# peaceminusones/Group-GAN-GCN-GAT

Measured on AMD Instinct MI355X. Metric: scenes/sec (obs8/pred12, 20 peds) at 1/2/4/8 GPUs; ADE/FDE vs ref, higher is better.
Workload: dtype fp32; 1 GPU; train iteration = D-step + G-step (best_k=20, Adam), GAT generator; BASELINE configs[1] shape (batch 64); scenes_per_gpu=64, global_batch=64, obs_len=8, pred_len=12, generator=gat, hip_graph=True, parallelism=dp1

## Files before the change

### group-gan-gcn-gat_amd/csrc/adam.hip

```cpp
#include "sgg_common.h"

namespace sgg {

constexpr int kAdamMaxTensors = 48;
constexpr int kAdamThreads = 256;
constexpr int kAdamChunk = 1024;

struct AdamList {
  float* p[kAdamMaxTensors];
  float* g[kAdamMaxTensors];
  float* m[kAdamMaxTensors];
  float* v[kAdamMaxTensors];
  float* step[kAdamMaxTensors];
  long long off[kAdamMaxTensors + 1];
  int n;
};

__device__ __forceinline__ float block_sum(float x, float* red) {
  for (int o = 32; o > 0; o >>= 1) x += __shfl_xor(x, o);
  const int lane = threadIdx.x & 63, wave = threadIdx.x >> 6;
  if (lane == 0) red[wave] = x;
  __syncthreads();
  float s = 0.f;
#pragma unroll
  for (int w = 0; w < kAdamThreads / 64; ++w) s += red[w];
  __syncthreads();
  return s;
}

constexpr int kAdamPer = kAdamChunk / kAdamThreads;

struct Tab {
  long long lo, hi;
  unsigned long long p, g, m, v;
};

__device__ __forceinline__ Tab lane_tab(const AdamList& L) {
  const int t = threadIdx.x & 63;
  Tab r = {0, 0, 0, 0, 0, 0};
  if (t < L.n) {
    r.lo = L.off[t];
    r.hi = L.off[t + 1];
    r.p = reinterpret_cast<unsigned long long>(L.p[t]);
    r.g = reinterpret_cast<unsigned long long>(L.g[t]);
    r.m = reinterpret_cast<unsigned long long>(L.m[t]);
    r.v = reinterpret_cast<unsigned long long>(L.v[t]);
  }
  return r;
}

__device__ __forceinline__ long long rl64(long long x, int k) {
  const int lo = __builtin_amdgcn_readlane((int)(unsigned)(unsigned long long)x, k);
  const int hi = __builtin_amdgcn_readlane((int)(unsigned)((unsigned long long)x >> 32), k);
  return (long long)(((unsigned long long)(unsigned)hi << 32) | (unsigned)lo);
}
__device__ __forceinline__ unsigned long long shfl64(unsigned long long x, int k) {
  const unsigned lo = (unsigned)__shfl((int)(unsigned)x, k), hi = (unsigned)__shfl((int)(unsigned)(x >> 32), k);
  return ((unsigned long long)hi << 32) | lo;
}

__device__ __forceinline__ void chunk_elems(const AdamList& L, const Tab& T, long long e0, int (&ek)[kAdamPer],
                                            long long (&ei)[kAdamPer]) {
  const long long total = L.off[L.n];
  const long long e1 = (e0 + kAdamChunk < total ? e0 + kAdamChunk : total) - 1;
  const int t = threadIdx.x & 63;
  const unsigned long long b0 = __ballot(t < L.n && T.lo <= e0 && e0 < T.hi);
  const unsigned long long b1 = __ballot(t < L.n && T.lo <= e1 && e1 < T.hi);
  const int k0 = b0 ? __ffsll((long long)b0) - 1 : 0, k1 = b1 ? __ffsll((long long)b1) - 1 : k0;
#pragma unroll
  for (int u = 0; u < kAdamPer; ++u) {
    ek[u] = -1;
    ei[u] = 0;
  }
  for (int k = k0; k <= k1; ++k) {
    const long long lo = rl64(T.lo, k), hi = rl64(T.hi, k);
#pragma unroll
    for (int u = 0; u < kAdamPer; ++u) {
      const long long e = e0 + threadIdx.x + (long long)u * kAdamThreads;
      if (e >= lo && e < hi) {
        ek[u] = k;
        ei[u] = e - lo;
      }
    }
  }
}

__global__ void __launch_bounds__(kAdamThreads) adam_prep_kernel(AdamList L, int clip, float* __restrict__ partial,
                                                                 float* __restrict__ scal, double lr, double beta1,
                                                                 double beta2) {
  __shared__ float red[kAdamThreads / 64];
  if (blockIdx.x == 0 && (int)threadIdx.x < L.n) {
    const float t = L.step[threadIdx.x][0] + 1.f;
    L.step[threadIdx.x][0] = t;
    scal[2 * threadIdx.x] = (float)(lr / (1.0 - pow(beta1, (double)t)));
    scal[2 * threadIdx.x + 1] = (float)sqrt(1.0 - pow(beta2, (double)t));
  }
  if (!clip) return;
  const long long e0 = (long long)blockIdx.x * kAdamChunk;
  const Tab T = lane_tab(L);
  int ek[kAdamPer];
  long long ei[kAdamPer];
  chunk_elems(L, T, e0, ek, ei);
  float x[kAdamPer];
#pragma unroll
  for (int u = 0; u < kAdamPer; ++u) {
    const float* g = reinterpret_cast<const float*>(shfl64(T.g, ek[u] < 0 ? 0 : ek[u]));
    x[u] = ek[u] >= 0 ? g[ei[u]] : 0.f;
  }
  float acc = 0.f;
#pragma unroll
  for (int u = 0; u < kAdamPer; ++u) acc = fmaf(x[u], x[u], acc);
  const float s = block_sum(acc, red);
  if (threadIdx.x == 0) partial[blockIdx.x] = s;
}

__global__ void __launch_bounds__(kAdamThreads) adam_update_kernel(AdamList L, int nparts, float max_norm,
                                                                   const float* __restrict__ partial,
                                                                   const float* __restrict__ scal, float beta2,
                                                                   float w1, float w2, float eps,
                                                                   unsigned* __restrict__ ticket, double lr,
                                                                   double beta1d, double beta2d) {
  __shared__ float red[kAdamThreads / 64];
  __shared__ int last;
  const long long e0 = (long long)blockIdx.x * kAdamChunk;
  const Tab T = lane_tab(L);
  float tstep = 0.f, lss = 0.f, lbc = 1.f;
  if (ticket && (int)(threadIdx.x & 63) < L.n) {
    tstep = L.step[threadIdx.x & 63][0] + 1.f;
    lss = (float)(lr / (1.0 - pow(beta1d, (double)tstep)));
    lbc = (float)sqrt(1.0 - pow(beta2d, (double)tstep));
  }
  int ek[kAdamPer];
  long long ei[kAdamPer];
  chunk_elems(L, T, e0, ek, ei);
  float coef = 1.f;
  if (max_norm > 0.f) {
    float acc = 0.f;
    for (int q = threadIdx.x; q < nparts; q += kAdamThreads) acc += partial[q];
    const float norm = sqrtf(block_sum(acc, red));
    coef = fminf(max_norm / (norm + 1e-6f), 1.f);
  }
  float* pp[kAdamPer];
  float* gp[kAdamPer];
  float* mp[kAdamPer];
  float* vp[kAdamPer];
  float gr[kAdamPer], m0[kAdamPer], v0[kAdamPer], p0[kAdamPer], ss[kAdamPer], bc[kAdamPer];
#pragma unroll
  for (int u = 0; u < kAdamPer; ++u) {
    const int k = ek[u] >= 0 ? ek[u] : 0;
    const long long i = ek[u] >= 0 ? ei[u] : 0;
    pp[u] = reinterpret_cast<float*>(shfl64(T.p, k)) + i;
    gp[u] = reinterpret_cast<float*>(shfl64(T.g, k)) + i;
    mp[u] = reinterpret_cast<float*>(shfl64(T.m, k)) + i;
    vp[u] = reinterpret_cast<float*>(shfl64(T.v, k)) + i;
    if (ticket) {
      ss[u] = __shfl(lss, k);
      bc[u] = __shfl(lbc, k);
    } else {
      ss[u] = scal[2 * k];
      bc[u] = scal[2 * k + 1];
    }
  }
#pragma unroll
  for (int u = 0; u < kAdamPer; ++u) {
    gr[u] = *gp[u];
    m0[u] = *mp[u];
    v0[u] = *vp[u];
    p0[u] = *pp[u];
  }
#pragma unroll
  for (int u = 0; u < kAdamPer; ++u) {
    if (ek[u] < 0) continue;
    float g = gr[u];
    if (max_norm > 0.f) {
      g *= coef;
      *gp[u] = g;
    }
    const float mi = m0[u] + w1 * (g - m0[u]);
    const float vi = v0[u] * beta2 + w2 * g * g;
    *mp[u] = mi;
    *vp[u] = vi;
    *pp[u] = p0[u] + -ss[u] * (mi / (sqrtf(vi) / bc[u] + eps));
  }
  if (ticket) {
    __syncthreads();
    if (threadIdx.x == 0) last = atomicAdd(ticket, 1u) == gridDim.x - 1;
    __syncthreads();
    if (last) {
      if ((int)threadIdx.x < L.n) L.step[threadIdx.x][0] = tstep;
      if (threadIdx.x == 0) *ticket = 0u;
    }
  }
}

}

using namespace sgg;

extern "C" int sgg_adam_parts(long long total) {
  return (int)((total + kAdamChunk - 1) / kAdamChunk) + 2 * kAdamMaxTensors + 1;
}

extern "C" int sgg_adam_step(float* const* params, float* const* grads, float* const* exp_avg,
                             float* const* exp_avg_sq, const long long* numel, int n, double lr, double beta1,
                             double beta2, float eps, float max_norm, float* const* step, float* ws,
                             size_t ws_bytes, void* stream) {
  SGG_CHECK_ARG(params && grads && exp_avg && exp_avg_sq && numel && step, "sgg_adam_step: null pointer");
  SGG_CHECK_ARG(n >= 1 && n <= kAdamMaxTensors, "sgg_adam_step: %d tensors (1..%d)", n, kAdamMaxTensors);
  AdamList L;
  L.n = n;
  L.off[0] = 0;
  for (int i = 0; i < n; ++i) {
    SGG_CHECK_ARG(params[i] && grads[i] && exp_avg[i] && exp_avg_sq[i] && step[i] && numel[i] >= 0,
                  "sgg_adam_step: tensor %d", i);
    L.p[i] = params[i];
    L.g[i] = grads[i];
    L.m[i] = exp_avg[i];
    L.v[i] = exp_avg_sq[i];
    L.step[i] = step[i];
    L.off[i + 1] = L.off[i] + numel[i];
  }
  const int parts = sgg_adam_parts(L.off[n]) - 2 * kAdamMaxTensors - 1;
  if (parts == 0) return 0;
  const int clip = max_norm > 0.f;
  SGG_CHECK_ARG(ws && ws_bytes >= sizeof(float) * ((size_t)parts + 2 * kAdamMaxTensors + 1),
                "sgg_adam_step: workspace");
  hipStream_t st = (hipStream_t)stream;
  unsigned* ticket = reinterpret_cast<unsigned*>(ws);
  float* partial = ws + 1;
  float* scal = partial + parts;
  if (clip)
    hipLaunchKernelGGL(adam_prep_kernel, dim3(parts), dim3(kAdamThreads), 0, st, L, clip, partial, scal, lr, beta1,
                       beta2);
  hipLaunchKernelGGL(adam_update_kernel, dim3(parts), dim3(kAdamThreads), 0, st, L, parts, clip ? max_norm : 0.f,
                     partial, scal, (float)beta2, (float)(1.0 - beta1), (float)(1.0 - beta2), eps, clip ? nullptr : ticket,
                     lr, beta1, beta2);
  SGG_RETURN_LAUNCH("sgg_adam_step");
}
```

### group-gan-gcn-gat_amd/csrc/fold.hip

```cpp
#include "sgg_common.h"

namespace sgg {

__global__ void __launch_bounds__(512) fold_fwd_kernel(const float* __restrict__ W, int ldw, int R, int E,
                                                       const float* __restrict__ We, const float* __restrict__ be,
                                                       const float* __restrict__ b1, const float* __restrict__ b2,
                                                       float* __restrict__ A, float* __restrict__ bias) {
  for (int r = threadIdx.x; r < R; r += blockDim.x) {
    float a0 = 0.f, a1 = 0.f, bb = 0.f;
    const float* w = W + (size_t)r * ldw;
#pragma unroll 8
    for (int e = 0; e < E; ++e) {
      const float we = w[e];
      a0 = fmaf(we, We[2 * e], a0);
      a1 = fmaf(we, We[2 * e + 1], a1);
      bb = fmaf(we, be[e], bb);
    }
    A[2 * r] = a0;
    A[2 * r + 1] = a1;
    bias[r] = bb + b1[r] + (b2 ? b2[r] : 0.f);
  }
}

struct FoldList {
  SggFold f[SGG_FOLD_MAX];
};

__global__ void __launch_bounds__(512) fold_fwd_multi_kernel(FoldList L) {
  const SggFold& d = L.f[blockIdx.x];
  for (int r = threadIdx.x; r < d.R; r += blockDim.x) {
    float a0 = 0.f, a1 = 0.f, bb = 0.f;
    const float* w = d.W + (size_t)r * d.ldw;
#pragma unroll 8
    for (int e = 0; e < d.E; ++e) {
      const float we = w[e];
      a0 = fmaf(we, d.We[2 * e], a0);
      a1 = fmaf(we, d.We[2 * e + 1], a1);
      bb = fmaf(we, d.be[e], bb);
    }
    d.A[2 * r] = a0;
    d.A[2 * r + 1] = a1;
    d.bias[r] = bb + d.b1[r] + (d.b2 ? d.b2[r] : 0.f);
  }
}

__device__ __forceinline__ void fold_bwd_body(const float* __restrict__ W, int ldw, int R, int E,
                                              const float* __restrict__ We, const float* __restrict__ be,
                                              const float* __restrict__ dA, const float* __restrict__ dbias,
                                              float* __restrict__ dW, int lddw, float* __restrict__ dWe,
                                              float* __restrict__ dbe, float* __restrict__ dbias_copy) {
  __shared__ float g3[3 * 512];
  __shared__ float part[3 * 512];
  for (int r = threadIdx.x; r < R; r += blockDim.x) {
    const float2 a = reinterpret_cast<const float2*>(dA)[r];
    const float b = dbias[r];
    g3[3 * r] = a.x;
    g3[3 * r + 1] = a.y;
    g3[3 * r + 2] = b;
    if (dbias_copy) dbias_copy[r] = b;
  }
  __syncthreads();
  const int ng = blockDim.x / E;
  const int t = threadIdx.x;
  if (t < ng * E) {
    const int e = t % E, g = t / E;
    const float we0 = We[2 * e], we1 = We[2 * e + 1], bee = be[e];
    float s0 = 0.f, s1 = 0.f, s2 = 0.f;
#pragma unroll 8
    for (int r = g; r < R; r += ng) {
      const float a0 = g3[3 * r], a1 = g3[3 * r + 1], b = g3[3 * r + 2];
      dW[(size_t)r * lddw + e] = fmaf(a0, we0, fmaf(a1, we1, b * bee));
      const float w = W[(size_t)r * ldw + e];
      s0 = fmaf(w, a0, s0);
      s1 = fmaf(w, a1, s1);
      s2 = fmaf(w, b, s2);
    }
    part[3 * t] = s0;
    part[3 * t + 1] = s1;
    part[3 * t + 2] = s2;
  }
  __syncthreads();
  if (t < 3 * E) {
    const int e = t / 3, j = t - 3 * e;
    float s = 0.f;
    for (int g = 0; g < ng; ++g) s += part[3 * (g * E + e) + j];
    if (j < 2) dWe[2 * e + j] = s;
    else dbe[e] = s;
  }
}

__global__ void __launch_bounds__(512) fold_bwd_kernel(const float* __restrict__ W, int ldw, int R, int E,
                                                       const float* __restrict__ We, const float* __restrict__ be,
                                                       const float* __restrict__ dA, const float* __restrict__ dbias,
                                                       float* __restrict__ dW, int lddw, float* __restrict__ dWe,
                                                       float* __restrict__ dbe, float* __restrict__ dbias_copy) {
  fold_bwd_body(W, ldw, R, E, We, be, dA, dbias, dW, lddw, dWe, dbe, dbias_copy);
}

struct FoldBwdList {
  SggFoldBwd f[SGG_FOLDB_MAX];
};

__global__ void __launch_bounds__(512) fold_bwd_multi_kernel(FoldBwdList L) {
  const SggFoldBwd& d = L.f[blockIdx.x];
  fold_bwd_body(d.W, d.ldw, d.R, d.E, d.We, d.be, d.dA_src, d.db_src, d.dW, d.lddw, d.dWe, d.dbe, d.dbias_copy);
}

void fold_bwd_multi(const SggFoldBwd* folds, int n, hipStream_t st) {
  FoldBwdList L;
  for (int k = 0; k < n; ++k) L.f[k] = folds[k];
  hipLaunchKernelGGL(fold_bwd_multi_kernel, dim3(n), dim3(512), 0, st, L);
}

}

using namespace sgg;

extern "C" int sgg_fold_fwd(const float* W, int ldw, int R, int E, const float* We, const float* be, const float* b1,
                            const float* b2, float* A, float* bias, void* stream) {
  SGG_CHECK_ARG(W && We && be && b1 && A && bias, "sgg_fold_fwd: null pointer");
  SGG_CHECK_ARG(R >= 1 && E >= 1 && ldw >= E, "sgg_fold_fwd: bad sizes R=%d E=%d ldw=%d", R, E, ldw);
  hipLaunchKernelGGL(fold_fwd_kernel, dim3(1), dim3(512), 0, (hipStream_t)stream, W, ldw, R, E, We, be, b1, b2, A,
                     bias);
  SGG_RETURN_LAUNCH("sgg_fold_fwd");
}

extern "C" int sgg_fold_fwd_multi(const SggFold* folds, int n, void* stream) {
  SGG_CHECK_ARG(folds && n >= 1 && n <= SGG_FOLD_MAX, "sgg_fold_fwd_multi: 1 <= n <= %d folds (got %d)", SGG_FOLD_MAX, n);
  FoldList L;
  for (int k = 0; k < n; ++k) {
    const SggFold& d = folds[k];
    SGG_CHECK_ARG(d.W && d.We && d.be && d.b1 && d.A && d.bias, "sgg_fold_fwd_multi: null pointer in fold %d", k);
    SGG_CHECK_ARG(d.R >= 1 && d.E >= 1 && d.ldw >= d.E, "sgg_fold_fwd_multi: bad sizes in fold %d", k);
    L.f[k] = d;
  }
  hipLaunchKernelGGL(fold_fwd_multi_kernel, dim3(n), dim3(512), 0, (hipStream_t)stream, L);
  SGG_RETURN_LAUNCH("sgg_fold_fwd_multi");
}

extern "C" int sgg_fold_bwd(const float* W, int ldw, int R, int E, const float* We, const float* be, const float* dA,
                            const float* dbias, float* dW, int lddw, float* dWe, float* dbe, float* dbias_copy,
                            void* stream) {
  SGG_CHECK_ARG(W && We && be && dA && dbias && dW && dWe && dbe, "sgg_fold_bwd: null pointer");
  SGG_CHECK_ARG(R >= 1 && R <= 512 && E >= 1 && E <= 128 && ldw >= E && lddw >= E, "sgg_fold_bwd: bad sizes");
  hipLaunchKernelGGL(fold_bwd_kernel, dim3(1), dim3(512), 0, (hipStream_t)stream, W, ldw, R, E, We, be, dA, dbias,
                     dW, lddw, dWe, dbe, dbias_copy);
  SGG_RETURN_LAUNCH("sgg_fold_bwd");
}
```

### group-gan-gcn-gat_amd/csrc/grad.hip

```cpp
#include <string.h>

#include "bce_body.h"
#include "sgg_common.h"

namespace sgg {

namespace {

constexpr int kRedJobs = SGG_RED_MAX + 2 * SGG_FOLDB_MAX;

struct FinishArgs {
  SggRed red[kRedJobs];
  unsigned char vec[kRedJobs];
  int nred;
  int blk0[kRedJobs + 1];
  SggL2Job l2[SGG_LOSSJOB_MAX];
  SggBceJob bce[SGG_LOSSJOB_MAX];
  int nl2, nbce;
};

__device__ __forceinline__ float phase_sum(const float* __restrict__ src, int rows, int ld, int col, int ph) {
  float s = 0.f;
  int r = ph;
  for (; r + 48 < rows; r += 64) {
    const float v0 = src[(size_t)r * ld + col], v1 = src[(size_t)(r + 16) * ld + col];
    const float v2 = src[(size_t)(r + 32) * ld + col], v3 = src[(size_t)(r + 48) * ld + col];
    s += v0;
    s += v1;
    s += v2;
    s += v3;
  }
  for (; r < rows; r += 16) s += src[(size_t)r * ld + col];
  return s;
}

__device__ __forceinline__ floatx4 phase_sum4(const float* __restrict__ src, int rows, int ld, int col, int ph) {
  floatx4 s = {0.f, 0.f, 0.f, 0.f};
  int r = ph;
  for (; r + 48 < rows; r += 64) {
    const floatx4 v0 = *reinterpret_cast<const floatx4*>(src + (size_t)r * ld + col);
    const floatx4 v1 = *reinterpret_cast<const floatx4*>(src + (size_t)(r + 16) * ld + col);
    const floatx4 v2 = *reinterpret_cast<const floatx4*>(src + (size_t)(r + 32) * ld + col);
    const floatx4 v3 = *reinterpret_cast<const floatx4*>(src + (size_t)(r + 48) * ld + col);
    s += v0;
    s += v1;
    s += v2;
    s += v3;
  }
  for (; r < rows; r += 16) s += *reinterpret_cast<const floatx4*>(src + (size_t)r * ld + col);
  return s;
}

__device__ __forceinline__ void red_store(const SggRed& d, int c, float v) {
  if (d.map == 0) {
    d.out[c] = v;
  } else {
    const int m = c / d.N, n = c - m * d.N;
    d.out[d.trans ? (size_t)n * d.ldo + m : (size_t)m * d.ldo + n] = v;
  }
}

__device__ void red_job(const SggRed& d, bool vec, int blk, float (*rpart)[256]) {
  const int el = threadIdx.x & 63, ph = threadIdx.x >> 6;
  if (vec) {
    const int c = blk * 256 + 4 * el;
    const floatx4 s = c < d.cols ? phase_sum4(d.src + d.col0, d.rows, d.ld, c, ph) : floatx4{0.f, 0.f, 0.f, 0.f};
    *reinterpret_cast<floatx4*>(&rpart[ph][4 * el]) = s;
    __syncthreads();
    if (ph == 0 && c < d.cols) {
      floatx4 v = {0.f, 0.f, 0.f, 0.f};
#pragma unroll
      for (int p = 0; p < 16; ++p) v += *reinterpret_cast<const floatx4*>(&rpart[p][4 * el]);
#pragma unroll
      for (int i = 0; i < 4; ++i)
        if (c + i < d.cols) red_store(d, c + i, v[i]);
    }
    return;
  }
  const int c = blk * 64 + el;
  const float s = c < d.cols ? phase_sum(d.src + d.col0, d.rows, d.ld, c, ph) : 0.f;
  rpart[ph][el] = s;
  __syncthreads();
  if (ph == 0 && c < d.cols) {
    float v = 0.f;
#pragma unroll
    for (int p = 0; p < 16; ++p) v += rpart[p][el];
    red_store(d, c, v);
  }
}

constexpr int kLossThreads = 1024;

__device__ void l2_value(const SggL2Job& d, float* lv) {
  if (threadIdx.x < 64) {
    float a = 0.f;
    for (int s = threadIdx.x; s < d.S; s += 64) a += d.term[s];
    a = wave_sum(a);
    if (threadIdx.x == 0) {
      *d.loss = a;
      *lv = a;
    }
  }
  __syncthreads();
}

static_assert(kLossThreads == kBceThreads, "the loss workgroup runs bce_value with its own thread count");

__device__ void loss_workgroup(const FinishArgs& a, float (*rpart)[256]) {
  __shared__ float lv[SGG_LOSSJOB_MAX];
  BceIn in[SGG_LOSSJOB_MAX];
#pragma unroll
  for (int j = 0; j < SGG_LOSSJOB_MAX; ++j)
    if (j < a.nbce) bce_load(a.bce[j], in[j]);
  float ad[SGG_LOSSJOB_MAX];
#pragma unroll
  for (int j = 0; j < SGG_LOSSJOB_MAX; ++j) {
    ad[j] = 0.f;
    if (j < a.nbce && a.bce[j].total) {
      bool fromL2 = false;
      for (int k = 0; k < a.nl2; ++k) fromL2 |= a.bce[j].addend == a.l2[k].loss;
      if (!fromL2) ad[j] = *a.bce[j].addend;
    }
  }
  for (int k = 0; k < a.nl2; ++k) l2_value(a.l2[k], lv + k);
#pragma unroll
  for (int j = 0; j < SGG_LOSSJOB_MAX; ++j)
    if (j < a.nbce) {
      float addend = ad[j];
      for (int k = 0; k < a.nl2; ++k)
        if (a.bce[j].total && a.bce[j].addend == a.l2[k].loss) addend = lv[k];
      bce_value(a.bce[j], in[j], addend, reinterpret_cast<float(*)[kLossThreads / 64]>(&rpart[0][0]));
    }
}

__global__ void __launch_bounds__(1024) grad_finish_kernel(FinishArgs a) {
  __shared__ __attribute__((aligned(16))) float rpart[16][256];
  const int lw = a.nl2 + a.nbce > 0;
  const int b = (int)blockIdx.x - lw;
  if (b < 0) {
    loss_workgroup(a, rpart);
    return;
  }
  int j = 0;
  while (j + 1 < a.nred && b >= a.blk0[j + 1]) ++j;
  red_job(a.red[j], a.vec[j] != 0, b - a.blk0[j], rpart);
}

}

}

using namespace sgg;

extern "C" int sgg_grad_finish(const SggRed* reds, int nred, const SggFoldBwd* folds, int nfold, float* scratch,
                               size_t scratch_bytes, void* stream) {
  return sgg_grad_finish_losses(reds, nred, folds, nfold, scratch, scratch_bytes, nullptr, 0, nullptr, 0, stream);
}

extern "C" int sgg_grad_finish_losses(const SggRed* reds, int nred, const SggFoldBwd* folds, int nfold,
                                      float* scratch, size_t scratch_bytes, const SggL2Job* l2, int nl2,
                                      const SggBceJob* bce, int nbce, void* stream) {
  SGG_CHECK_ARG(nl2 >= 0 && nl2 <= SGG_LOSSJOB_MAX && nbce >= 0 && nbce <= SGG_LOSSJOB_MAX &&
                    (nl2 == 0 || l2) && (nbce == 0 || bce),
                "sgg_grad_finish_losses: 0 <= nl2, nbce <= %d (got %d, %d)", SGG_LOSSJOB_MAX, nl2, nbce);
  for (int j = 0; j < nl2; ++j) {
    const SggL2Job& d = l2[j];
    SGG_CHECK_ARG(d.loss && (d.S == 0 || d.term) && d.S >= 0, "sgg_grad_finish_losses: bad L2 job %d", j);
  }
  for (int j = 0; j < nbce; ++j) {
    const SggBceJob& d = bce[j];
    SGG_CHECK_ARG(d.ya && d.yb && d.loss && (d.n == 0 || d.x) && (!d.total || d.addend),
                  "sgg_grad_finish_losses: null pointer in BCE job %d", j);
    SGG_CHECK_ARG(d.n >= 0 && d.split >= 0 && d.split <= d.n, "sgg_grad_finish_losses: BCE job %d: bad sizes", j);
  }
  SGG_CHECK_ARG(nred >= 0 && nred <= SGG_RED_MAX && nfold >= 0 && nfold <= SGG_FOLDB_MAX,
                "sgg_grad_finish: 0 <= nred <= %d, 0 <= nfold <= %d (got %d, %d)", SGG_RED_MAX, SGG_FOLDB_MAX, nred,
                nfold);
  SGG_CHECK_ARG((nred == 0 || reds) && (nfold == 0 || (folds && scratch)), "sgg_grad_finish: null job list or scratch");
  FinishArgs a;
  memset(&a, 0, sizeof(a));
  int nj = 0;
  auto add_red = [&](const SggRed& d) {
    a.red[nj] = d;
    ++nj;
  };
  for (int j = 0; j < nred; ++j) {
    const SggRed& d = reds[j];
    SGG_CHECK_ARG(d.src && d.out && d.rows >= 0 && d.cols >= 1 && d.col0 >= 0 && d.ld >= d.col0 + d.cols,
                  "sgg_grad_finish: bad reduction job %d (rows %d ld %d col0 %d cols %d)", j, d.rows, d.ld, d.col0,
                  d.cols);
    SGG_CHECK_ARG(d.map == 0 || (d.map == 1 && d.N >= 1 && d.cols % d.N == 0 &&
                                 d.ldo >= (d.trans ? d.cols / d.N : d.N)),
                  "sgg_grad_finish: bad output map of reduction job %d", j);
    add_red(d);
  }
  size_t need = 0;
  for (int k = 0; k < nfold; ++k) need += sizeof(float) * 3 * (size_t)folds[k].R;
  SGG_CHECK_ARG(scratch_bytes >= need, "sgg_grad_finish: scratch %zu < %zu bytes", scratch_bytes, need);
  float* g = scratch;
  for (int k = 0; k < nfold; ++k) {
    const SggFoldBwd& d = folds[k];
    SGG_CHECK_ARG(d.W && d.We && d.be && d.dA_src && d.db_src && d.dW && d.dWe && d.dbe,
                  "sgg_grad_finish: null pointer in fold job %d", k);
    SGG_CHECK_ARG(d.R >= 1 && d.R <= 512 && d.E >= 1 && d.E <= 128 && d.ldw >= d.E && d.lddw >= d.E,
                  "sgg_grad_finish: bad fold sizes in job %d (R %d E %d)", k, d.R, d.E);
    SGG_CHECK_ARG(d.dA_rows >= 0 && d.db_rows >= 0 && d.dA_col0 >= 0 && d.db_col0 >= 0 &&
                      d.dA_ld >= d.dA_col0 + 2 * d.R && d.db_ld >= d.db_col0 + d.R,
                  "sgg_grad_finish: bad (dA, dbias) sources in fold job %d", k);
    add_red(SggRed{d.dA_src, d.dA_rows, d.dA_ld, d.dA_col0, 2 * d.R, g, 0, 0, 0, 0});
    add_red(SggRed{d.db_src, d.db_rows, d.db_ld, d.db_col0, d.R, g + 2 * d.R, 0, 0, 0, 0});
    g += 3 * (size_t)d.R;
  }
  a.nred = nj;
  int blk = 0;
  for (int j = 0; j < nj; ++j) {
    const SggRed& d = a.red[j];
    a.vec[j] = d.ld % 4 == 0 && d.col0 % 4 == 0 && (reinterpret_cast<uintptr_t>(d.src) & 15) == 0;
    a.blk0[j] = blk;
    blk += a.vec[j] ? (d.cols + 255) / 256 : (d.cols + 63) / 64;
  }
  a.blk0[nj] = blk;
  for (int j = 0; j < nl2; ++j) a.l2[j] = l2[j];
  for (int j = 0; j < nbce; ++j) a.bce[j] = bce[j];
  a.nl2 = nl2;
  a.nbce = nbce;
  if (nl2 + nbce > 0) ++blk;
  hipStream_t st = (hipStream_t)stream;
  if (blk > 0) hipLaunchKernelGGL(grad_finish_kernel, dim3(blk), dim3(1024), 0, st, a);
  if (nfold > 0) {
    SggFoldBwd f[SGG_FOLDB_MAX];
    g = scratch;
    for (int k = 0; k < nfold; ++k) {
      f[k] = folds[k];
      f[k].dA_src = g;
      f[k].db_src = g + 2 * folds[k].R;
      g += 3 * (size_t)folds[k].R;
    }
    fold_bwd_multi(f, nfold, st);
  }
  SGG_RETURN_LAUNCH("sgg_grad_finish");
}
```

### group-gan-gcn-gat_amd/sgan/_native.py

```python
import ctypes
import os

import torch

from ._srchash import source_hash

_LIB_EXPLICIT = bool(os.environ.get("SGG_LIB"))
_LIB_PATH = os.environ.get("SGG_LIB") or os.path.join(os.path.dirname(os.path.abspath(__file__)), "_lib", "libsgg.so")

_i = ctypes.c_int
_f = ctypes.c_float
_p = ctypes.c_void_p
_sz = ctypes.c_size_t
_u = ctypes.c_uint
_u64 = ctypes.c_ulonglong

MAX_HEADS = 4


class GatEncWeights(ctypes.Structure):
    _fields_ = [("Wi", _p * MAX_HEADS), ("ai", _p * MAX_HEADS), ("Wio", _p), ("aio", _p),
                ("Wg", _p * MAX_HEADS), ("ag", _p * MAX_HEADS), ("Wgo", _p), ("ago", _p), ("Woe", _p), ("boe", _p)]


class GatEncArgs(ctypes.Structure):
    _fields_ = [("X", _p), ("ldx", _i), ("labels", _p), ("scene_off", _p), ("S", _i), ("np", _i), ("nh", _i),
                ("alpha", _f), ("w", GatEncWeights), ("y", _p), ("ldy", _i), ("dy", _p), ("lddy", _i), ("dX", _p),
                ("lddx", _i), ("slab", _p), ("saved", _p), ("X2", _p), ("ldx2", _i), ("kx1", _i),
                ("dX2", _p), ("lddx2", _i), ("dy_copies", _i), ("dy_cstride", _i)]


_pargs = ctypes.POINTER(GatEncArgs)


class GcnModArgs(ctypes.Structure):
    _fields_ = [("X", _p), ("ldx", _i), ("X2", _p), ("ldx2", _i), ("kx1", _i), ("labels", _p), ("scene_off", _p),
                ("S", _i), ("np", _i), ("fin", _i), ("fe", _i), ("bf16", _i), ("W0i", _p), ("W1i", _p), ("W0g", _p),
                ("W1g", _p), ("Woe", _p), ("boe", _p), ("y", _p), ("ldy", _i), ("dy", _p), ("lddy", _i),
                ("dy_copies", _i), ("dy_cstride", _i), ("dX", _p), ("lddx", _i), ("dX2", _p), ("lddx2", _i),
                ("slab", _p)]


_gargs = ctypes.POINTER(GcnModArgs)


class LstmSeg(ctypes.Structure):
    _fields_ = [("rel", _p), ("A", _p), ("Whh", _p), ("bias", _p), ("h0", _p), ("c0", _p), ("T", _i), ("B", _i),
                ("Bl", _i), ("t0", _i), ("Tl", _i), ("Bsrc", _i), ("h_all", _p), ("c_all", _p), ("act_all", _p),
                ("Wu", _p), ("ldwu", _i), ("cu", _p), ("NU", _i), ("U", _p)]


_sargs = ctypes.POINTER(LstmSeg)


class PoolDh(ctypes.Structure):
    _fields_ = [("dU", _p), ("ldu", _i), ("W1h", _p), ("ldw", _i), ("base", _p), ("NU", _i), ("h", _p), ("ldh", _i),
                ("ws", _p), ("ws_bytes", _sz), ("splits", _i)]


GLUE_NONE, GLUE_SELECT, GLUE_L2BWD = 0, 1, 2


class GlueSeg(ctypes.Structure):
    _fields_ = [("kind", _i), ("pred", _p), ("ldp", _i), ("gt", _p), ("mask", _p), ("ldm", _i), ("scene_off", _p),
                ("S", _i), ("T", _i), ("B", _i), ("k", _i), ("best", _p), ("w", _f), ("gout", _p), ("dpred", _p),
                ("ldd", _i), ("term", _p)]

FOLD_MAX = 8


class Fold(ctypes.Structure):
    _fields_ = [("W", _p), ("ldw", _i), ("R", _i), ("E", _i), ("We", _p), ("be", _p), ("b1", _p), ("b2", _p),
                ("A", _p), ("bias", _p)]

RED_MAX = 24
FOLDB_MAX = 6


class Red(ctypes.Structure):
    _fields_ = [("src", _p), ("rows", _i), ("ld", _i), ("col0", _i), ("cols", _i), ("out", _p), ("map", _i),
                ("N", _i), ("ldo", _i), ("trans", _i)]


class FoldBwd(ctypes.Structure):
    _fields_ = [("W", _p), ("ldw", _i), ("R", _i), ("E", _i), ("We", _p), ("be", _p),
                ("dA_src", _p), ("dA_rows", _i), ("dA_ld", _i), ("dA_col0", _i),
                ("db_src", _p), ("db_rows", _i), ("db_ld", _i), ("db_col0", _i),
                ("dW", _p), ("lddw", _i), ("dWe", _p), ("dbe", _p), ("dbias_copy", _p)]


class DecInit(ctypes.Structure):
    _fields_ = [("ctx", _p), ("ldc", _i), ("Dc", _i), ("z", _p), ("nz", _i), ("best", _p), ("first_k", _i),
                ("ped_scene", _p), ("S", _i), ("Bper", _i), ("last_rel", _p)]


LOSSJOB_MAX = 2


class TrajOut(ctypes.Structure):
    _fields_ = [("out", _p), ("NB", _i), ("T0", _i), ("col0", _i), ("ncol", _i), ("head", _p), ("ldh", _i),
                ("b", _p), ("ldb", _i), ("pos0", _p), ("start", _p)]


class PoolBatch(ctypes.Structure):
    _fields_ = [("U", _p), ("pos", _p), ("scene_off", _p), ("chunks", _p), ("nchunks", _i), ("max_rows", _i),
                ("gpw", _i), ("B", _i), ("max_n", _i), ("out", _p), ("argmax", _p), ("nchunks_dev", _p)]


class GatLayerSet(ctypes.Structure):
    _fields_ = [("x1", _p), ("ld1", _i), ("K1", _i), ("x2", _p), ("ld2", _i), ("K2", _i), ("seg_off", _p),
                ("nseg", _i), ("n", _i), ("max_seg", _i), ("xn", _p), ("rstd", _p), ("wh", _p), ("hp", _p), ("y", _p),
                ("ldy", _i)]


class L2Job(ctypes.Structure):
    _fields_ = [("term", _p), ("S", _i), ("loss", _p)]


class BceJob(ctypes.Structure):
    _fields_ = [("x", _p), ("n", _i), ("split", _i), ("ya", _p), ("yb", _p), ("w", _f), ("loss", _p),
                ("addend", _p), ("total", _p), ("nvalid", _p)]


class DecStep(ctypes.Structure):
    _fields_ = ([(n, _i) for n in ("B", "H", "bn", "mlp_dim", "NU", "mlp", "cell", "ldwu")]
                + [(n, _p) for n in ("h_prev", "pool_prev", "c_prev", "r_in", "pos_prev",
                                     "W1m", "b1m", "W2m", "b2m", "A", "Whh", "bias", "Wp", "bp", "Wu", "cu",
                                     "h", "c", "rel", "pos", "U", "act", "h_mix", "z1")])


class DecStepBwd(ctypes.Structure):
    _fields_ = ([(n, _i) for n in ("B", "H", "bn", "mlp_dim", "mlp", "cell")]
                + [(n, _p) for n in ("dh", "dc", "drel", "dpos", "act", "c", "c_prev", "h_mix", "z1",
                                     "W1m", "W2m", "A", "Whh", "Wp",
                                     "dh_prev", "dpool_prev", "dc_prev", "dr_in", "dpos_prev",
                                     "dG", "dz2", "dz1", "drel_tot")])


SIGNATURES = {
    "sgg_version": (_i, []),
    "sgg_last_error": (ctypes.c_char_p, []),
    "sgg_source_hash": (ctypes.c_char_p, []),
    "sgg_xw": (_i, [_p, _i, _p, _i, _p, _i, _i, _p, _p, _i, _i, _i, _i, _i, _p]),
    "sgg_xw_bf16": (_i, [_p, _i, _p, _i, _p, _i, _i, _p, _p, _i, _i, _i, _i, _i, _p]),
    "sgg_pool_plan": (_i, [_p, _i, _i, _i, _i, _p, _i, _p, _p]),
    "sgg_pool_fwd": (_i, [_p, _p, _p, _p, _p, _p, _p, _i, _i, _i, _i, _i, _i, _p, _p, _p, _p]),
    "sgg_pool_plan_bf16": (_i, [_p, _i, _i, _i, _p, _i, _p, _p]),
    "sgg_pool_fwd_bf16": (_i, [_p, _p, _p, _p, _p, _p, _p, _i, _i, _i, _i, _i, _i, _p, _p, _p, _p]),
    "sgg_pool_fwd2": (_i, [ctypes.POINTER(PoolBatch), ctypes.POINTER(PoolBatch), _p, _p, _p, _i, _i, _p]),
    "sgg_pool_bwd_grid": (_i, [_i]),
    "sgg_pool_dh_dw": (_i, [_p, _i, _p, _i, _p, _i, _i, _p, _i, _i, _i, _p, _sz, _p]),
    "sgg_pool_bwd": (_i, [_p, _p, _p, _p, _p, _p, _p, _p, _i, _i, _i, _i, _p, _p, _p]),
    "sgg_pool_plan_wide": (_i, [_p, _i, _i, _i, _p, _i, _p, _p]),
    "sgg_pool_fwd_wide": (_i, [_p, _p, _p, _p, _p, _p, _p, _i, _i, _i, _i, _i, _i, _p, _p, _p]),
    "sgg_pool_bwd_wide_grid": (_i, [_i, _i]),
    "sgg_pool_bwd_wide": (_i, [_p, _p, _p, _p, _p, _p, _p, _p, _i, _i, _i, _i, _p, _p, _p]),
    "sgg_pool_plan_bn": (_i, [_p, _i, _i, _i, _p, _i, _p, _p]),
    "sgg_pool_fwd_bn": (_i, [_p, _p, _p, _p, _p, _p, _p, _i, _i, _i, _i, _i, _i, _p, _p, _p]),
    "sgg_pool_bwd_bn_grid": (_i, [_i, _i, _i]),
    "sgg_pool_bwd_bn_ws_floats": (ctypes.c_longlong, [_i, _i, _i, _i]),
    "sgg_pool_bwd_bn": (_i, [_p, _p, _p, _p, _p, _p, _p, _p, _i, _i, _i, _i, _p, _p, _sz, _p]),
    "sgg_gat_fwd": (_i, [_p, _i, _p, _p, _p, _p, _i, _i, _i, _f, _i, _i, _i, _p, _p, _i, _p]),
    "sgg_gat_bwd": (_i, [_p, _i, _p, _p, _p, _i, _i, _i, _f, _i, _i, _i, _p, _p, _p, _i, _p, _p, _p, _p]),
    "sgg_gat_fwd_ex": (_i, [_p, _i, _p, _p, _p, _p, _p, _i, _i, _i, _f, _i, _i, _i, _p, _p, _i, _p]),
    "sgg_gat_bwd_ex": (_i, [_p, _i, _p, _p, _p, _p, _i, _i, _i, _f, _i, _i, _i, _p, _p, _p, _i, _p, _p, _p, _p, _p,
                            _p]),
    "sgg_gat_bwd_ex_work_bytes": (_sz, [_i, _i, _i]),
    "sgg_gat_wide_work_floats": (_sz, [_i, _i, _i, _i, _i]),
    "sgg_gat_fwd_wide": (_i, [_p, _i, _p, _p, _i, _p, _p, _p, _i, _i, _i, _f, _i, _i, _i, _p, _p, _i, _p, _p]),
    "sgg_gat_bwd_wide": (_i, [_p, _i, _p, _p, _i, _p, _p, _i, _i, _i, _f, _i, _i, _i, _p, _p, _p, _i, _p, _p, _p, _p,
                              _p, _p, _p, _p]),
    "sgg_gat_fwd_drop": (_i, [_p, _i, _p, _p, _i, _p, _p, _p, _i, _i, _i, _f, _i, _i, _i, _p, _p, _i,
                              _f, _u64, _u, _u, _u, _p, _p]),
    "sgg_gat_bwd_drop": (_i, [_p, _i, _p, _p, _i, _p, _p, _i, _i, _i, _f, _i, _i, _i, _p, _p, _p, _i, _p, _p, _p, _p,
                              _p, _p, _p, _f, _u64, _u, _u, _u, _p, _p]),
    "sgg_dropout": (_i, [_p, _i, _i, _i, _f, _u64, _u, _u, _p, _p, _i, _p]),
    "sgg_gat_layer_lds_bytes": (_sz, [_i, _i, _i]),
    "sgg_gat_layer_fwd": (_i, [_p, _i, _i, _p, _i, _i, _p, _p, _p, _p, _p, _i, _i, _i, _i, _f, _f, _i, _i, _i, _p, _p,
                               _p, _p, _p, _i, _p]),
    "sgg_gat_layer_fwd2": (_i, [ctypes.POINTER(GatLayerSet), ctypes.POINTER(GatLayerSet), _p, _p, _p, _p, _i, _i, _f,
                                _f, _i, _i, _p]),
    "sgg_seg_norm_fwd": (_i, [_p, _i, _i, _p, _i, _f, _p, _i, _p, _p]),
    "sgg_seg_norm_bwd": (_i, [_p, _i, _p, _i, _i, _p, _i, _p, _p, _i, _p]),
    "sgg_group_index_ws": (_sz, [_i, _i]),
    "sgg_group_index": (_i, [_p, _p, _i, _i, _i, _p, _p, _p, _p, _p, _p, _p]),
    "sgg_seg_reduce": (_i, [_p, _i, _i, _p, _p, _p, _p, _p, _i, _i, _p, _i, _p]),
    "sgg_seg_gather": (_i, [_p, _i, _i, _p, _p, _p, _i, _p, _i, _p]),
    "sgg_xtw_splits": (_i, [_i, _i, _i]),
    "sgg_lstm_bwd_split": (_i, [_p, _p, _p, _p, _p, _p, _p, _p, _p, _p, _i, _i, _i, _i, _p, _p, _p, _p, _p]),
    "sgg_lstm_bwd_tail": (_i, [_p, _p, _p, _p, _p, _p, _p, _i, _i, _i, _i, _p, _p]),
    "sgg_lstm_fwd_seg": (_i, [_sargs, _i, _p]),
    "sgg_lstm_fwd_seg_glue": (_i, [_sargs, _i, ctypes.POINTER(GlueSeg), _p]),
    "sgg_lstm_fwd_seg2": (_i, [_sargs, _i, _sargs, _i, _p]),
    "sgg_lstm_fwd_seg3": (_i, [_sargs, _i, _sargs, _i, _sargs, _i, _p]),
    "sgg_lstm_bwd_shared": (_i, [_p, _p, _p, _p, _p, _p, _p, _i, _i, _i, _i, _i, _p, _p, _p]),
    "sgg_lstm_bwd_pooldh_ok": (_i, [_i]),
    "sgg_lstm_bwd_pooldh_pays": (_i, [_i, _i]),
    "sgg_lstm_bwd_pooldh_rides": (_i, [_i, _i, _i]),
    "sgg_lstm_bwd_pooldh": (_i, [_p, _p, _p, _p, _p, _p, ctypes.POINTER(PoolDh), _i, _i, _i, _i, _i, _i, _p, _p, _p,
                                 _p]),
    "sgg_lstm_u_ok": (_i, [_i, _i, _i, _i, _i, _i]),
    "sgg_lstm_fwd_u": (_i, [_p, _p, _p, _p, _p, _p, _i, _i, _i, _p, _p, _p, _p, _i, _p, _i, _p, _p]),
    "sgg_head_ok": (_i, [_i, _i]),
    "sgg_head_slab_cols": (_i, [_i, _i]),
    "sgg_head_fwd": (_i, [_p, _i, _i, _i, _i, _p, _p, _p, _p, _i, _p, _p, _p]),
    "sgg_head_bwd": (_i, [_p, _i, _i, _i, _i, _p, _p, _p, _p, _p, _i, _p, _i, _p, _p, _p, _p, _i, _f, _p, _p]),
    "sgg_head_fwdbwd": (_i, [_p, _i, _i, _i, _i, _p, _p, _p, _p, _i, _p, _p, _i, _p, _p, _p, _p, _i, _f, _p, _p]),
    "sgg_xtw_partial": (_i, [_p, _i, _p, _i, _p, _i, _i, _i, _i, _i, _p, _sz, _p]),
    "sgg_grad_finish": (_i, [ctypes.POINTER(Red), _i, ctypes.POINTER(FoldBwd), _i, _p, _sz, _p]),
    "sgg_lstm_fwd_dec": (_i, [ctypes.POINTER(DecInit), _p, _p, _p, _p, _p, _i, _i, _i, _p, _p, _p, _p, _p,
                              ctypes.POINTER(TrajOut), _p]),
    "sgg_lstm_fwd_dec2": (_i, [ctypes.POINTER(DecInit), ctypes.POINTER(DecInit), _p, _p, _p, _p, _p, _i, _i, _i, _i,
                               _p, _p, ctypes.POINTER(TrajOut), _p]),
    "sgg_lstm_fwd_dec_seg": (_i, [ctypes.POINTER(DecInit), _p, _p, _p, _p, _p, _i, _i, _i, _p, _p, _p, _p, _p,
                                  ctypes.POINTER(TrajOut), _sargs, _i, _p]),
    "sgg_grad_finish_losses": (_i, [ctypes.POINTER(Red), _i, ctypes.POINTER(FoldBwd), _i, _p, _sz,
                                    ctypes.POINTER(L2Job), _i, ctypes.POINTER(BceJob), _i, _p]),
    "sgg_adam_parts": (_i, [ctypes.c_longlong]),
    "sgg_adam_step": (_i, [_p, _p, _p, _p, _p, _i, ctypes.c_double, ctypes.c_double, ctypes.c_double, _f, _f, _p, _p,
                          _sz, _p]),
    "sgg_xtw": (_i, [_p, _i, _p, _i, _p, _i, _i, _i, _i, _p, _i, _i, _p, _p, _sz, _p]),
    "sgg_fold_fwd": (_i, [_p, _i, _i, _i, _p, _p, _p, _p, _p, _p, _p]),
    "sgg_fold_fwd_multi": (_i, [ctypes.POINTER(Fold), _i, _p]),
    "sgg_fold_bwd": (_i, [_p, _i, _i, _i, _p, _p, _p, _p, _p, _i, _p, _p, _p, _p]),
    "sgg_lstm_fwd": (_i, [_p, _p, _p, _p, _p, _p, _p, _p, _i, _i, _i, _i, _p, _p, _p, _p, _p]),
    "sgg_lstm_state_floats": (ctypes.c_longlong, [_i, _i, _i, _i]),
    "sgg_lstm_dg_floats": (ctypes.c_longlong, [_i, _i, _i]),
    "sgg_lstm_wpart_rows": (_i, [_i, _i]),
    "sgg_lstm_kernel_name": (ctypes.c_char_p, [_i, _i, _i, _i, _i]),
    "sgg_lstm_bwd": (_i, [_p, _p, _p, _p, _p, _p, _p, _p, _p, _p, _i, _i, _i, _i, _p, _p, _p, _p, _p, _p]),
    "sgg_bce_fwd": (_i, [_p, _i, _i, _p, _p, _f, _p, _p, _p, _p, _p]),
    "sgg_bce_bwd": (_i, [_p, _i, _i, _p, _p, _f, _p, _p, _p, _p]),
    "sgg_gatenc_param_size": (_i, [_i]),
    "sgg_gatenc_lds_bytes": (ctypes.c_longlong, [_i, _i, _i]),
    "sgg_gatenc_saved_floats": (ctypes.c_longlong, [_i, _i, _i]),
    "sgg_gatenc_fwd": (_i, [_pargs, _p]),
    "sgg_gatenc_fwd2": (_i, [_pargs, _pargs, _p]),
    "sgg_gatenc_bwd": (_i, [_pargs, _p]),
    "sgg_gcnmod_param_size": (_i, [_i, _i]),
    "sgg_gcnmod_slab_rows": (_i, [_i]),
    "sgg_gcnmod_lds_bytes": (ctypes.c_longlong, [_i, _i, _i, _i]),
    "sgg_gcnmod_fwd": (_i, [_gargs, _p]),
    "sgg_gcnmod_fwd2": (_i, [_gargs, _gargs, _p]),
    "sgg_gcnmod_bwd": (_i, [_gargs, _p]),
    "sgg_slab_reduce": (_i, [_p, _i, _i, _p, _p]),
    "sgg_gather_batch_floats": (ctypes.c_longlong, [_i, _i, _i]),
    "sgg_gather_batch": (_i, [_p, _i, _p, _i, _i, _i, _p, _p]),
    "sgg_traj_cat": (_i, [_p, _i, _i, _p, _i, _p, _i, _i, _i, _p, _p, _p, _p]),
    "sgg_decoder_init": (_i, [_p, _i, _i, _p, _i, _p, _i, _i, _p, _i, _i, _p, _p, _p, _p]),
    "sgg_l2_select": (_i, [_p, _p, _p, _i, _p, _i, _i, _i, _i, _p, _p]),
    "sgg_l2_loss_fwd": (_i, [_p, _i, _p, _p, _i, _p, _i, _i, _i, _f, _p, _p, _p, _p]),
    "sgg_l2_loss_bwd": (_i, [_p, _i, _p, _p, _i, _p, _p, _i, _i, _f, _p, _p, _i, _p]),
    "sgg_l2_loss_bwd_scenes": (_i, [_p, _i, _p, _p, _i, _p, _i, _i, _i, _f, _p, _p, _i, _p, _p]),
    "sgg_val_metrics_work_floats": (_sz, [_i]),
    "sgg_val_metrics": (_i, [_p, _p, _p, _p, _p, _i, _p, _p, _f, _i, _i, _p, _p, _p]),
    "sgg_dec_step_ok": (_i, [_i, _i, _i, _i]),
    "sgg_dec_step_saved_floats": (ctypes.c_longlong, [_i, _i, _i]),
    "sgg_dec_step_fwd": (_i, [ctypes.POINTER(DecStep), _p]),
    "sgg_dec_step_bwd": (_i, [ctypes.POINTER(DecStepBwd), _p]),
    "sgg_pool_dpos": (_i, [_p, _p, _p, _p, _p, _p, _p, _p, _i, _i, _i, _p, _p]),
    "sgg_pool_fwd_bn_drop": (_i, [_p, _p, _p, _p, _p, _p, _p, _i, _i, _i, _i, _i, _i, _p, _p, _f, _u64, _u, _p, _p]),
    "sgg_pool_bwd_bn_drop": (_i, [_p, _p, _p, _p, _p, _p, _p, _p, _i, _i, _i, _i, _p, _p, _sz, _f, _u64, _u, _p, _p]),
    "sgg_pool_dpos_drop": (_i, [_p, _p, _p, _p, _p, _p, _p, _p, _i, _i, _i, _p, _f, _u64, _u, _p, _p]),
    "sgg_pool_norm_fwd": (_i, [_p] * 10 + [_i] * 5 + [_f, _f] + [_p] * 9),
    "sgg_pool_norm_running": (_i, [_p, _p, _p, _i, _i, _f, _p, _p, _p]),
    "sgg_pool_norm_bwd_rows": (_i, [_i]),
    "sgg_pool_norm_bwd_ws_floats": (ctypes.c_longlong, [_i, _i, _i]),
    "sgg_pool_norm_bwd_slab_offset": (ctypes.c_longlong, [_i, _i]),
    "sgg_pool_norm_bwd": (_i, [_p] * 18 + [_i] * 5 + [_f, _f, _i, _p, _p, _p, _sz, _p]),
}

VAL_SLOTS = 11

_lib = None


class NativeError(RuntimeError):
    pass


def lib_path():
    return _LIB_PATH


def built_hash():
    return load(require_gpu=False).sgg_source_hash().decode()


def load(require_gpu=True):
    global _lib
    if _lib is None:
        if not os.path.exists(_LIB_PATH):
            raise NativeError("libsgg.so not built at %s -- run group-gan-gcn-gat_amd/build_native.py "
                              "(or __graft_entry__.build())" % _LIB_PATH)
        lib = ctypes.CDLL(_LIB_PATH)
        for name, (res, args) in SIGNATURES.items():
            fn = getattr(lib, name)
            fn.restype = res
            fn.argtypes = args
        if not _LIB_EXPLICIT:
            built, tree = lib.sgg_source_hash().decode(), source_hash()
            if built != tree:
                raise NativeError("%s was built from other sources (hash %s) than this tree's csrc/ + "
                                  "include/sgg.h (%s) -- rebuild with group-gan-gcn-gat_amd/build_native.py"
                                  % (_LIB_PATH, built[:16], tree[:16]))
        _lib = lib
    if require_gpu and not torch.cuda.is_available():
        raise NativeError("sgan: no HIP device visible; the MI355X kernels have no CPU fallback")
    return _lib


def check(rc, name):
    if rc != 0:
        msg = _lib.sgg_last_error().decode(errors="replace")
        raise NativeError("%s failed (rc=%d): %s" % (name, rc, msg))


def stream_ptr():
    return ctypes.c_void_p(torch.cuda.current_stream().cuda_stream)


def ptr(t):
    if t is None:
        return None
    return ctypes.c_void_p(t.data_ptr())
```

### group-gan-gcn-gat_amd/sgan/kernels.py

```python
import collections
import contextlib
import ctypes
import functools
import os
import weakref

import torch

from . import _native as N

GATENC_FUSED = os.environ.get("SGG_GATENC_FUSED", "1") != "0"
GATENC_SAVE = os.environ.get("SGG_GATENC_SAVE", "1") != "0"
DUAL_POOL_BWD = os.environ.get("SGG_DUAL_POOL_BWD", "1") != "0"
POOL_DH_IN_LSTM = os.environ.get("SGG_POOL_DH_IN_LSTM", "1") != "0"


DEBUG = os.environ.get("SGG_DEBUG", "0") == "1"


def _lib():
    return N.load()


def _req(t, name, dtype=torch.float32):
# ... 46 lines not shown
    import ctypes
    dev = torch.cuda.current_device() if device is None else torch.device(device).index
    if dev is None:
        dev = torch.cuda.current_device()
    key = (tag, dev)
    st = _private.get(key)
    if st is None:
        if _hiprt is None:
            lib = ctypes.CDLL(os.path.join(os.path.dirname(torch.__file__), "lib", "libamdhip64.so"))
            lib.hipStreamCreateWithFlags.argtypes = [ctypes.POINTER(ctypes.c_void_p), ctypes.c_uint]
            lib.hipStreamCreateWithFlags.restype = ctypes.c_int
            _hiprt = lib
        h = ctypes.c_void_p()
        with torch.cuda.device(dev):
            rc = _hiprt.hipStreamCreateWithFlags(ctypes.byref(h), 1)
        if rc != 0 or not h.value:
            raise N.NativeError("hipStreamCreateWithFlags failed (%d)" % rc)
        st = _private[key] = torch.cuda.ExternalStream(h.value, device=torch.device("cuda", dev))
    return st


def xw_raw(x, w, bias=None, trans_w=False, act=0, out=None, mask=None, prec=None):
    x = _rows(x, "x")
    if mask is not None:
        mask = _rows(mask, "mask")
        assert mask.shape == x.shape
    w = _rows(w, "w")
    M, K = x.shape
    Nn = w.shape[0] if trans_w else w.shape[1]
    assert (w.shape[1] if trans_w else w.shape[0]) == K, (x.shape, w.shape, trans_w)
    if bias is not None:
        bias = _req(bias, "bias").contiguous()
        assert bias.numel() == Nn
    y = out if out is not None else torch.empty(M, Nn, device=x.device, dtype=torch.float32)

    bf16 = (prec or _PRECISION) == "bf16"
    fn = _lib().sgg_xw_bf16 if bf16 else _lib().sgg_xw

    def launch():
        N.check(fn(N.ptr(x), x.stride(0), N.ptr(mask), mask.stride(0) if mask is not None else 0,
                   N.ptr(w), w.stride(0), int(bool(trans_w)), N.ptr(bias), N.ptr(y), y.stride(0), M, K, Nn,
                   int(act), N.stream_ptr()), "sgg_xw")
    launch()
    if timer.active and M > 0:
        tw = "true" if trans_w else "false"
        name = ("sgg::xw_bf16_kernel<%s>" % tw if bf16 else
                "sgg::xw_splitk_kernel<%s>" % tw if K >= 256 else
                "sgg::xw_kernel<true, true>" if trans_w and K <= 256 else
                "sgg::xw_kernel<%s, false>" % tw)
        timer.add(name, (M, K, Nn, mask is not None), 2.0 * M * K * Nn,
                  4.0 * (M * K * (2 if mask is not None else 1) + K * Nn + M * Nn), launch)
    return y


def xtw(X, Y, colsum=False, trans_c=False, out=None, mask=None):
    lib = _lib()
    X = _rows(X, "X")
    Y = _rows(Y, "Y")
    if mask is not None:
        mask = _rows(mask, "mask")
        assert mask.shape == Y.shape
    R, M = X.shape
    Nn = Y.shape[1]
    assert Y.shape[0] == R
    shape = (Nn, M) if trans_c else (M, Nn)
    if out is None:
        C = torch.empty(shape, device=X.device, dtype=torch.float32)
    else:
        assert tuple(out.shape) == shape and out.stride(1) == 1, (out.shape, shape)
        C = out
    if R == 0:
        C.zero_()
        return (C, torch.zeros(Nn, device=X.device)) if colsum else C
    splits = lib.sgg_xtw_splits(R, M, Nn)
    ws = torch.empty(splits * (M * Nn + Nn), device=X.device, dtype=torch.float32)
    cs = torch.empty(Nn, device=X.device, dtype=torch.float32) if colsum else None
    def launch():
        N.check(lib.sgg_xtw(N.ptr(X), X.stride(0), N.ptr(Y), Y.stride(0), N.ptr(mask),
                            mask.stride(0) if mask is not None else 0, R, M, Nn, N.ptr(C), C.stride(0), int(trans_c),
                            N.ptr(cs), N.ptr(ws), ws.numel() * 4, N.stream_ptr()), "sgg_xtw")
    launch()
    if timer.active:
        timer.add("sgg::xtw_partial_kernel+xtw_reduce_kernel", (R, M, Nn, mask is not None), 2.0 * R * M * Nn,
                  4.0 * (R * M + R * Nn * (2 if mask is not None else 1) + M * Nn) + 8.0 * ws.numel(), launch)
    return (C, cs) if colsum else C


def fold_fwd(W, We, be, b1, b2=None):
    key, ver = _fold_key(W, We, be, b1, b2)
    ent = _FOLD_CACHE.get(key)
    if _fold_hit(ent, ver, (W, We, be, b1, b2)):
        return ent[1], ent[2]
    prefold([(W, We, be, b1, b2)])
    ent = _FOLD_CACHE[key]
    return ent[1], ent[2]


_EPOCH = {}
_FOLD_CACHE = {}


def _fold_key(W, We, be, b1, b2):
    ts = (W, We, be, b1, b2)
    key = tuple((t.data_ptr(), tuple(t.shape), t.stride(0)) if t is not None else None for t in ts)
    ver = tuple((t._version, _EPOCH.get(t.data_ptr(), 0)) if t is not None else None for t in ts)
    return key, ver


def _owner(t):
    return t._base if t._base is not None else t


def _fold_hit(ent, ver, ts):
    return (ent is not None and ent[0] == ver
            and all((r is None) if t is None else (r is not None and r() is _owner(t)) for r, t in zip(ent[4], ts)))


def _fold_purge():
    dead = [k for k, e in _FOLD_CACHE.items() if any(r is not None and r() is None for r in e[4])]
    for k in dead:
        del _FOLD_CACHE[k]


def clear_fold_cache():
    _FOLD_CACHE.clear()


def prefold(specs):
    todo = []
    for W, We, be, b1, b2 in specs:
        key, ver = _fold_key(W, We, be, b1, b2)
        if not _fold_hit(_FOLD_CACHE.get(key), ver, (W, We, be, b1, b2)):
            todo.append((key, ver, (W, We, be, b1, b2)))
    if not todo:
        return
    _fold_purge()
    arr = (N.Fold * len(todo))()
    outs = []
    for k, (key, ver, (W, We, be, b1, b2)) in enumerate(todo):
        W = _rows(W, "W")
        R, E = W.shape
        A = torch.empty(R, 2, device=W.device, dtype=torch.float32)
        bias = torch.empty(R, device=W.device, dtype=torch.float32)
        parts = (W, We.contiguous(), be.contiguous(), b1.contiguous(), b2.contiguous() if b2 is not None else None)
        arr[k] = N.Fold(N.ptr(parts[0]), W.stride(0), R, E, N.ptr(parts[1]), N.ptr(parts[2]), N.ptr(parts[3]),
                        N.ptr(parts[4]), N.ptr(A), N.ptr(bias))
        outs.append((key, ver, A, bias, parts))
    for i in range(0, len(todo), N.FOLD_MAX):
        chunk = (N.Fold * min(N.FOLD_MAX, len(todo) - i))(*arr[i:i + N.FOLD_MAX])
        N.check(_lib().sgg_fold_fwd_multi(chunk, len(chunk), N.stream_ptr()), "sgg_fold_fwd_multi")
    for (key, ver, A, bias, parts), (_, _, ts) in zip(outs, todo):
        refs = tuple(weakref.ref(_owner(t)) if t is not None else None for t in ts)
        copies = tuple(p for p, t in zip(parts, ts) if p is not None and p.data_ptr() != t.data_ptr())
        _FOLD_CACHE[key] = (ver, A, bias, copies, refs)


def lstm_fold_spec(lstm, emb):
    return (lstm.weight_ih_l0, emb.weight, emb.bias, lstm.bias_ih_l0, lstm.bias_hh_l0)


def pool_fold_spec(pool):
    l1, E = pool_linears(pool)[0], pool.embedding_dim
    return (l1.weight[:, :E], pool.spatial_embedding.weight, pool.spatial_embedding.bias, l1.bias, None)


def fold_bwd(W, We, be, dA, dbias, dW=None, dbias_copy=None):
    W = _rows(W, "W")
    R, E = W.shape
    dW = dW if dW is not None else torch.empty(R, E, device=W.device, dtype=torch.float32)
    dWe = torch.empty(E, 2, device=W.device, dtype=torch.float32)
    dbe = torch.empty(E, device=W.device, dtype=torch.float32)
    N.check(_lib().sgg_fold_bwd(N.ptr(W), W.stride(0), R, E, N.ptr(We.contiguous()), N.ptr(be.contiguous()),
                                N.ptr(dA.contiguous()), N.ptr(dbias.contiguous()), N.ptr(dW), dW.stride(0), N.ptr(dWe),
                                N.ptr(dbe), N.ptr(dbias_copy), N.stream_ptr()), "sgg_fold_bwd")
    return dW, dWe, dbe


def xtw_partial(X, Y, colsum=False):
    lib = _lib()
    X = _rows(X, "X")
    Y = _rows(Y, "Y")
    R, M = X.shape
    Nn = Y.shape[1]
    assert Y.shape[0] == R and R > 0
    splits = lib.sgg_xtw_splits(R, M, Nn)
    ws = torch.empty(splits * (M * Nn + (Nn if colsum else 0)), device=X.device, dtype=torch.float32)

    def launch():
        N.check(lib.sgg_xtw_partial(N.ptr(X), X.stride(0), N.ptr(Y), Y.stride(0), None, 0, R, M, Nn, int(colsum),
                                    N.ptr(ws), ws.numel() * 4, N.stream_ptr()), "sgg_xtw_partial")
    launch()
    if timer.active:
        mt = 4 if M >= 64 else (M + 15) // 16
        timer.add("sgg::xtw_partial_kernel<%d>" % mt, (R, M, Nn), 2.0 * R * M * Nn,
                  4.0 * (R * M + R * Nn) + 4.0 * ws.numel(), launch)
    return ws, splits


class GradFinish:

    def __init__(self):
        self.reds, self.folds, self.keep = [], [], []

    def _hold(self, *ts):
        self.keep += [t.untyped_storage() for t in ts if t is not None]

    def rowsum(self, src, rows, ld, col0, cols, out):
        assert out.is_contiguous() and out.numel() == cols
        self.reds.append(N.Red(N.ptr(src), rows, ld, col0, cols, N.ptr(out), 0, 0, 0, 0))
        self._hold(src, out)

    def xtw_sums(self, ws, splits, M, Nn, C, trans_c=False, colsum=None):
        assert C.stride(1) == 1 and tuple(C.shape) == ((Nn, M) if trans_c else (M, Nn))
        self.reds.append(N.Red(N.ptr(ws), splits, M * Nn, 0, M * Nn, N.ptr(C), 1, Nn, C.stride(0), int(trans_c)))
        self._hold(ws, C)
        if colsum is not None:
            self.rowsum(ws[splits * M * Nn:], splits, Nn, 0, Nn, colsum)

    def fold(self, W, We, be, dA_src, dA_rows, dA_ld, dA_col0, db_src, db_rows, db_ld, db_col0, dW=None,
             dbias_copy=None):
        W = _rows(W, "W")
        R, E = W.shape
        dW = dW if dW is not None else torch.empty(R, E, device=W.device, dtype=torch.float32)
        dWe = torch.empty(E, 2, device=W.device, dtype=torch.float32)
        dbe = torch.empty(E, device=W.device, dtype=torch.float32)
        We, be = We.contiguous(), be.contiguous()
        self.folds.append(N.FoldBwd(N.ptr(W), W.stride(0), R, E, N.ptr(We), N.ptr(be),
                                    N.ptr(dA_src), dA_rows, dA_ld, dA_col0, N.ptr(db_src), db_rows, db_ld, db_col0,
                                    N.ptr(dW), dW.stride(0), N.ptr(dWe), N.ptr(dbe), N.ptr(dbias_copy)))
        self._hold(W, We, be, dA_src, db_src, dW, dWe, dbe, dbias_copy)
        return dW, dWe, dbe

    def run(self):
        if not self.reds and not self.folds:
            return
        if _DEFER[0] > 0:
            _PENDING.append(self)
            return
        _finish_launch(self.reds, self.folds, self.keep)


_DEFER = [0]
_PENDING = []
_LOSS = {"l2": [], "bce": [], "keep": [], "out": set()}


DEFER_LOSSES = os.environ.get("SGG_DEFER_LOSSES", "1") != "0"


def _loss_deferrable(kind):
    return DEFER_LOSSES and _DEFER[0] > 0 and not _NO_DEFER[0] and len(_LOSS[kind]) < N.LOSSJOB_MAX


@contextlib.contextmanager
def eager_losses():
    prev = _NO_DEFER[0]
    _NO_DEFER[0] = True
    try:
        yield
    finally:
        _NO_DEFER[0] = prev


_NO_DEFER = [False]


def _queue_loss(kind, job, keep, outs):
    _LOSS[kind].append(job)
    _LOSS["keep"] += [t.untyped_storage() for t in keep if t is not None]
    _LOSS["out"].update(t.data_ptr() for t in outs)


def _loss_pending(t):
    return t is not None and t.data_ptr() in _LOSS["out"]


def _take_losses():
    glue_flush()
    l2, bce, keep = _LOSS["l2"], _LOSS["bce"], _LOSS["keep"]
    _LOSS.update(l2=[], bce=[], keep=[], out=set())
    return l2, bce, keep


def flush_losses():
    l2, bce, keep = _take_losses()
    if l2 or bce:
        _finish_launch([], [], keep, l2, bce)


@contextlib.contextmanager
def defer_grad_finish():
    if os.environ.get("SGG_CHECK_DEFER") == "1":
        yield
        return
    _DEFER[0] += 1
    try:
        yield
    finally:
        _DEFER[0] -= 1
        if _DEFER[0] == 0:
            grad_flush()


def grad_flush():
    if not _PENDING:
        flush_losses()
    while _PENDING:
        reds, folds, keep = [], [], []
        while _PENDING and len(reds) + len(_PENDING[0].reds) <= N.RED_MAX \
                and len(folds) + len(_PENDING[0].folds) <= N.FOLDB_MAX:
            gf = _PENDING.pop(0)
            reds += gf.reds
            folds += gf.folds
            keep += gf.keep
        if not reds and not folds:
            raise N.NativeError("grad_flush: a queued finish exceeds the job limits")
        l2, bce = [], []
        if not _PENDING:
            l2, bce, lkeep = _take_losses()
            keep = keep + lkeep
        _finish_launch(reds, folds, keep, l2, bce)


def _finish_launch(reds_l, folds_l, keep, l2_l=(), bce_l=()):
    lib = _lib()
    assert len(reds_l) <= N.RED_MAX and len(folds_l) <= N.FOLDB_MAX
    assert len(l2_l) <= N.LOSSJOB_MAX and len(bce_l) <= N.LOSSJOB_MAX
    reds = (N.Red * max(1, len(reds_l)))(*reds_l)
    folds = (N.FoldBwd * max(1, len(folds_l)))(*folds_l)
    l2 = (N.L2Job * max(1, len(l2_l)))(*l2_l)
    bce = (N.BceJob * max(1, len(bce_l)))(*bce_l)
    nr, nf, nl, nb = len(reds_l), len(folds_l), len(l2_l), len(bce_l)
    dev = keep[0].device
    scratch = torch.empty(max(1, sum(3 * f.R for f in folds_l)), device=dev, dtype=torch.float32)

    def launch(reds=reds, folds=folds, nr=nr, nf=nf, l2=l2, bce=bce, nl=nl, nb=nb, keep=list(keep)):
        N.check(lib.sgg_grad_finish_losses(reds, nr, folds, nf, N.ptr(scratch), scratch.numel() * 4, l2, nl, bce, nb,
                                           N.stream_ptr()), "sgg_grad_finish")
    launch()
    if timer.active:
        nb = sum(4.0 * r.rows * r.cols for r in reds_l) + sum(4.0 * 3 * f.R * max(f.dA_rows, f.db_rows)
                                                               for f in folds_l)
        timer.add("sgg::grad_finish_kernel", (nr, nf, tuple((r.rows, r.cols) for r in reds_l)), nb / 4.0, nb,
                  launch)


class _XW(torch.autograd.Function):
    @staticmethod
    def forward(ctx, x, w, bias, trans_w, act):
        y = xw_raw(x, w, bias, trans_w, act)
        ctx.trans_w, ctx.act, ctx.has_bias = trans_w, act, bias is not None
        ctx.save_for_backward(x, w, y if act else None)
        return y

    @staticmethod
    def backward(ctx, dy):
        x, w, y = ctx.saved_tensors
        dy = dy.contiguous()
        m = y if ctx.act else None
        dx = dw = db = None
        if ctx.needs_input_grad[0]:
            dx = xw_raw(dy, w, None, not ctx.trans_w, 0, mask=m, prec="fp32")
        if ctx.needs_input_grad[1] or (ctx.has_bias and ctx.needs_input_grad[2]):
            dw, cs = xtw(x, dy, colsum=True, trans_c=ctx.trans_w, mask=m)
            db = cs if ctx.has_bias else None
        return dx, dw, db, None, None


def xw(x, w, bias=None, trans_w=False, act=0):
    return _XW.apply(x, w, bias, trans_w, act)


def linear(x, lin, act=0):
    return _XW.apply(x, lin.weight, lin.bias, True, act)


def head_ok(seq):
    mods = list(seq)
    lins = [m for m in mods if isinstance(m, torch.nn.Linear)]
    if len(lins) != 2 or any(not isinstance(m, (torch.nn.Linear, torch.nn.ReLU)) for m in mods):
        return None
    l1, l2 = lins
    if l2.out_features != 1 or l1.bias is None or l2.bias is None:
        return None
    if not _lib().sgg_head_ok(l1.in_features, l1.out_features):
        return None
    i1, i2 = mods.index(l1), mods.index(l2)
    relu1 = i1 + 1 < len(mods) and isinstance(mods[i1 + 1], torch.nn.ReLU)
    relu2 = i2 + 1 < len(mods) and isinstance(mods[i2 + 1], torch.nn.ReLU)
    if len(mods) != 2 + int(relu1) + int(relu2):
        return None
    return l1, l2, int(relu1) | (2 * int(relu2))


class BceLink:

    def __init__(self):
        self.pending = None
        self.forward_held = None
        self.fused = None

    def put(self, g, ya, yb, split, w, placeholder, nvalid=None):
        self.pending = (g, ya, yb, split, w, placeholder, nvalid)

    def take(self):
        p, self.pending = self.pending, None
        return p

    def run_fused(self, ya, yb, split, w, nvalid):
        held, self.forward_held = self.forward_held, None
        if held is None:
            return
        x, W1, b1, W2, b2, act, y, wgrad = held
        lib = _lib()
        M, Kd = x.shape
        N1 = W1.shape[0]
        seed = const(1.0, x.device)
        dx = torch.empty(M, Kd, device=x.device, dtype=torch.float32)
        P = lib.sgg_head_slab_cols(Kd, N1)
        slab = torch.empty(max((M + 63) // 64, 1), P, device=x.device, dtype=torch.float32) if wgrad else None

        def launch():
            N.check(lib.sgg_head_fwdbwd(N.ptr(x), x.stride(0), M, Kd, N1, N.ptr(W1), N.ptr(b1), N.ptr(W2), N.ptr(b2),
                                        act, N.ptr(y), N.ptr(dx), dx.stride(0), N.ptr(slab), N.ptr(seed), N.ptr(ya),
                                        N.ptr(yb), int(split), float(w), N.ptr(nvalid), N.stream_ptr()),
                    "sgg_head_fwdbwd")
        launch()
        if timer.active and M > 0:
            timer.add("sgg::head_fwdbwd_kernel<%d, %d>" % (N1 // 16, Kd // 16), (M, Kd, N1, wgrad),
                      2.0 * M * N1 * (Kd + 1) + 2.0 * M * N1 * Kd * (2 if wgrad else 1),
                      4.0 * (M * Kd * (2 if wgrad else 1) + N1 * Kd + 2 * M + M * Kd
                             + (slab.numel() if wgrad else 0)), launch)
        self.fused = (seed, dx, slab)

    def flush_forward(self):
        held, self.forward_held = self.forward_held, None
        if held is not None:
            x, W1, b1, W2, b2, act, y, _ = held
            _head_fwd(x, W1, b1, W2, b2, act, y, record=True)


HEAD_FUSE = os.environ.get("SGG_HEAD_FUSE", "1") != "0"
_HELD_HEADS = []


def _head_fwd(x, W1, b1, W2, b2, act, y, record=False):
    lib = _lib()
    M, Kd = x.shape
    N1 = W1.shape[0]
    hid = torch.empty(M, N1, device=x.device, dtype=torch.float32)

    def launch():
        N.check(lib.sgg_head_fwd(N.ptr(x), x.stride(0), M, Kd, N1, N.ptr(W1), N.ptr(b1), N.ptr(W2), N.ptr(b2),
                                 act, N.ptr(hid), N.ptr(y), N.stream_ptr()), "sgg_head_fwd")
    launch()
    if record and timer.active and M > 0:
        timer.add("sgg::head_fwd_kernel<%d, %d>" % (N1 // 16, Kd // 16), (M, Kd, N1), 2.0 * M * N1 * (Kd + 1),
                  4.0 * (M * Kd + N1 * Kd + M * N1 + M), launch)
    return hid


class _Head(torch.autograd.Function):
    @staticmethod
    def forward(ctx, x, W1, b1, W2, b2, act, bce_link=None):
        x = _rows(x, "x")
        if x.data_ptr() % 16 or x.stride(0) % 4:
            x = x.contiguous()
        M, Kd = x.shape
        W1, W2 = W1.contiguous(), W2.contiguous()
        b1, b2 = b1.contiguous(), b2.contiguous()
        y = torch.empty(M, 1, device=x.device, dtype=torch.float32)
        wgrad = any(ctx.needs_input_grad[1:5])
        if bce_link is not None and HEAD_FUSE and M > 0:
            bce_link.forward_held = (x, W1, b1, W2, b2, act, y, wgrad)
            _HELD_HEADS.append(bce_link)
            hid = None
        else:
            hid = _head_fwd(x, W1, b1, W2, b2, act, y, record=True)
        ctx.act = act
        ctx.bce_link = bce_link
        ctx.hid = hid
        ctx.save_for_backward(x, W1, b1, W2, b2, y)
        return y

    @staticmethod
    def backward(ctx, dy):
        lib = _lib()
        x, W1, b1, W2, b2, y = ctx.saved_tensors
        need = ctx.needs_input_grad
        M, Kd = x.shape
        N1 = W1.shape[0]
        link = ctx.bce_link
        pend = link.take() if link is not None else None
        if link is not None and link.forward_held is not None:
            link.flush_forward()
        fused, hid = None, ctx.hid
        if link is not None and link.fused is not None:
            fused, link.fused = link.fused, None
        bce = None
        if pend is not None:
            g, ya, yb, split, w, ph, nvalid = pend
            if dy.data_ptr() != ph.data_ptr():
                raise N.NativeError("fused head + BCE backward: the scores have a consumer besides the BCE loss "
                                    "(set SGG_HEAD_BCE=0)")
            bce = (g.contiguous(), ya, yb, int(split), float(w), nvalid)
        else:
            dy = dy.contiguous()
        wgrad = any(need[1:5])
        P = lib.sgg_head_slab_cols(Kd, N1)
        rows = (M + 63) // 64
        if fused is not None and bce is not None and bce[0].data_ptr() == fused[0].data_ptr():
            dx, slab = fused[1], fused[2]
        else:
            if hid is None:
                hid = _head_fwd(x, W1, b1, W2, b2, ctx.act, torch.empty_like(y))
            dx = torch.empty(M, Kd, device=x.device, dtype=torch.float32)
            slab = torch.empty(max(rows, 1), P, device=x.device, dtype=torch.float32) if wgrad else None
            bg, bya, byb, bsp, bw, bnv = (N.ptr(bce[0]), N.ptr(bce[1]), N.ptr(bce[2]), bce[3], bce[4],
                                          N.ptr(bce[5])) if bce else (None, None, None, 0, 0.0, None)

            def launch():
                N.check(lib.sgg_head_bwd(N.ptr(x), x.stride(0), M, Kd, N1, N.ptr(W1), N.ptr(W2), N.ptr(hid),
                                         N.ptr(y), None if bce else N.ptr(dy), ctx.act, N.ptr(dx), dx.stride(0),
                                         N.ptr(slab), bg, bya, byb, bsp, bw, bnv, N.stream_ptr()), "sgg_head_bwd")
            launch()
            if timer.active and M > 0:
                timer.add("sgg::head_bwd_kernel<%d, %d>" % (N1 // 16, Kd // 16), (M, Kd, N1, wgrad),
                          2.0 * M * N1 * Kd * (2 if wgrad else 1),
                          4.0 * (M * Kd * (3 if wgrad else 2) + 2 * M * N1 + (slab.numel() if wgrad else 0)), launch)
        ctx.hid = None
        if not wgrad:
            return dx, None, None, None, None, None, None
        dW1 = torch.empty(N1, Kd, device=x.device, dtype=torch.float32)
        db1 = torch.empty(N1, device=x.device, dtype=torch.float32)
        dW2 = torch.empty(1, N1, device=x.device, dtype=torch.float32)
        db2 = torch.empty(1, device=x.device, dtype=torch.float32)
        if M == 0:
            for t in (dW1, db1, dW2, db2):
                t.zero_()
        else:
            gf = GradFinish()
            gf.rowsum(slab, rows, P, 0, N1 * Kd, dW1)
            gf.rowsum(slab, rows, P, N1 * Kd, N1, db1)
            gf.rowsum(slab, rows, P, N1 * Kd + N1, N1, dW2)
            gf.rowsum(slab, rows, P, N1 * Kd + 2 * N1, 1, db2)
            gf.run()
        return dx, dW1, db1, dW2, db2, None, None


HEAD_BCE = os.environ.get("SGG_HEAD_BCE", "1") != "0"
_BCE_HANDOFF = [0]


@contextlib.contextmanager
def bce_handoff():
    _BCE_HANDOFF[0] += 1
    try:
        yield
    finally:
        _BCE_HANDOFF[0] -= 1
        if _BCE_HANDOFF[0] == 0:
            while _HELD_HEADS:
                _HELD_HEADS.pop().flush_forward()


def head(x, spec):
    l1, l2, act = spec
    link = BceLink() if (HEAD_BCE and _BCE_HANDOFF[0] > 0 and torch.is_grad_enabled()) else None
    y = _Head.apply(x, l1.weight, l1.bias, l2.weight, l2.bias, act, link)
    if link is not None:
        y._sgg_bce_link = link
    return y


class ClipAdam:

    MAX_TENSORS = 48

    def __init__(self, params, lr, betas=(0.9, 0.999), eps=1e-8):
        self.params = [p for p in params]
        self.opt = torch.optim.Adam(self.params, lr=lr, betas=betas, eps=eps, capturable=True)
        self._ws = None

    def _state(self, p):
        st = self.opt.state[p]
        if "exp_avg" not in st:
            st["step"] = torch.zeros((), dtype=torch.float32, device=p.device)
            st["exp_avg"] = torch.zeros_like(p, memory_format=torch.preserve_format)
            st["exp_avg_sq"] = torch.zeros_like(p, memory_format=torch.preserve_format)
        elif not torch.is_tensor(st["step"]) or st["step"].device != p.device or st["step"].dtype != torch.float32:
            st["step"] = torch.as_tensor(float(st["step"]), dtype=torch.float32).to(p.device)
        return st

    @property
    def param_groups(self):
        return self.opt.param_groups

    def state_dict(self):
        return self.opt.state_dict()

    def load_state_dict(self, sd):
        self.opt.load_state_dict(sd)
        for p in self.params:
            if self.opt.state.get(p):
                self._state(p)

    def zero_grad(self, set_to_none=True):
        self.opt.zero_grad(set_to_none=set_to_none)

    def step(self, max_norm=0.0):
        lib = _lib()
        grp = self.opt.param_groups[0]
        act = [p for p in self.params if p.grad is not None]
        if max_norm > 0:
            self._launch(lib, act, grp, max_norm)
            return
        for i in range(0, len(act), self.MAX_TENSORS):
            self._launch(lib, act[i:i + self.MAX_TENSORS], grp, 0.0)

    def _launch(self, lib, act, grp, max_norm):
        import ctypes
        if len(act) > self.MAX_TENSORS:
            raise N.NativeError("ClipAdam: %d tensors with gradients, the fused step takes <= %d (clipping needs "
                              "them in one call)" % (len(act), self.MAX_TENSORS))
        for p in act:
            for t in (p, p.grad):
                if t.dtype != torch.float32 or not t.is_contiguous() or not t.is_cuda:
                    raise N.NativeError("ClipAdam: parameters and grads must be contiguous fp32 device tensors")
        n = len(act)
        st = [self._state(p) for p in act]
        for p in act:
            _EPOCH[p.data_ptr()] = _EPOCH.get(p.data_ptr(), 0) + 1
        arr = lambda xs: (ctypes.c_void_p * n)(*[x.data_ptr() for x in xs])
        numel = (ctypes.c_longlong * n)(*[p.numel() for p in act])
        total = sum(p.numel() for p in act)
        parts = lib.sgg_adam_parts(total)
        if self._ws is None or self._ws.numel() < parts:
            self._ws = torch.zeros(parts, device=act[0].device, dtype=torch.float32)
        b1, b2 = grp["betas"]
        N.check(lib.sgg_adam_step(arr(act), arr([p.grad for p in act]), arr([s["exp_avg"] for s in st]),
                                  arr([s["exp_avg_sq"] for s in st]), numel, n, float(grp["lr"]), float(b1),
                                  float(b2), float(grp["eps"]), float(max_norm), arr([s["step"] for s in st]),
                                  N.ptr(self._ws), self._ws.numel() * 4, N.stream_ptr()), "sgg_adam_step")


class OwnershipError(N.NativeError):
    """A re-issuable launch holds a raw device pointer (inside a ctypes
    descriptor) to memory it does not keep alive."""


def _storage_span(obj):
    s = obj.untyped_storage() if isinstance(obj, torch.Tensor) else obj
    b = s.data_ptr()
    return (b, b + s.nbytes())


def _walk_held(obj, spans, descs, seen, depth=0):
    import ctypes
    if obj is None or isinstance(obj, (int, float, str, bytes, bool)) or depth > 6 or id(obj) in seen:
        return
    seen.add(id(obj))
    if isinstance(obj, (torch.Tensor, torch.UntypedStorage)):
        sp = _storage_span(obj)
        if sp is not None:
            spans.append(sp)
        return
    if isinstance(obj, (ctypes.Structure, ctypes.Array)):
        descs.append(obj)
        for v in getattr(obj, "__dict__", {}).values():
            _walk_held(v, spans, descs, seen, depth + 1)
        return
    if isinstance(obj, (list, tuple, set, frozenset)):
        for v in obj:
            _walk_held(v, spans, descs, seen, depth + 1)
        return
    if isinstance(obj, dict):
        for v in obj.values():
            _walk_held(v, spans, descs, seen, depth + 1)
        return
    if isinstance(obj, functools.partial):
        for v in (obj.func, obj.args, obj.keywords):
            _walk_held(v, spans, descs, seen, depth + 1)
        return
    code = getattr(obj, "__code__", None)
    if code is not None:
        for c in obj.__closure__ or ():
            try:
                _walk_held(c.cell_contents, spans, descs, seen, depth + 1)
            except ValueError:
                pass
        _walk_held(obj.__defaults__, spans, descs, seen, depth + 1)
        _walk_held(obj.__kwdefaults__, spans, descs, seen, depth + 1)
        return
    if hasattr(obj, "__self__") and hasattr(obj, "__func__"):
        _walk_held(obj.__self__, spans, descs, seen, depth + 1)
        return
    d = getattr(obj, "__dict__", None)
    if d is not None and not isinstance(obj, (type, torch.nn.Module)):
        _walk_held(d, spans, descs, seen, depth + 1)


def _desc_pointers(desc, path="", out=None):
    import ctypes
    out = [] if out is None else out
    if isinstance(desc, ctypes.Array):
        for i in range(len(desc)):
            v = desc[i]
            if isinstance(v, (ctypes.Structure, ctypes.Array)):
                _desc_pointers(v, "%s[%d]" % (path, i), out)
            elif desc._type_ is ctypes.c_void_p and v:
                out.append(("%s[%d]" % (path, i), v))
        return out
    for fname, ftype in desc._fields_:
        v = getattr(desc, fname)
        if isinstance(v, (ctypes.Structure, ctypes.Array)):
            _desc_pointers(v, path + "." + fname, out)
        elif ftype is ctypes.c_void_p and v:
            out.append((path + "." + fname, v))
    return out


def check_ownership(fn, name="launch"):
    spans, descs = [], []
    _walk_held(fn, spans, descs, set())
    spans.sort()
    for d in descs:
        for path, p in _desc_pointers(d, type(d).__name__):
            if not any(b <= p < e for b, e in spans):
                raise OwnershipError("%s: descriptor field %s points to 0x%x, which the re-issuable launch does "
                                     "not keep alive" % (name, path, p))


@contextlib.contextmanager
def capture_guard():
    import gc
    gc.collect()
    was = gc.isenabled()
    gc.disable()
    try:
        yield
    finally:
        if was:
            gc.enable()


def capture_error_mode():
    import torch.distributed as dist
    return "thread_local" if dist.is_available() and dist.is_initialized() else "global"


@contextlib.contextmanager
def gc_frozen():
    import gc
    own = gc.get_freeze_count() == 0
    if own:
        gc.collect()
        gc.freeze()
    try:
        yield
    finally:
        if own:
            gc.unfreeze()


class LaunchTimer:

    def __init__(self):
        self.active = False
        self.rec = []

    def start(self):
        self.active, self.rec = True, []

    def stop(self):
        self.active = False
        torch.cuda.synchronize()
        out, self.rec = self.rec, []
        return out

    def add(self, name, key, flop, nbytes, relaunch):
        if self.active:
            check_ownership(relaunch, name)
            self.rec.append((name, (name,) + tuple(key), float(flop), float(nbytes), relaunch))

    @staticmethod
    def replay(records, reps=20):
        with capture_guard():
            return LaunchTimer._replay(records, reps)

    @staticmethod
    def _replay(records, reps):
        res = {}
        cur = torch.cuda.current_stream()
        for name, key, fl, nb, fn in records:
            if key in res:
                res[key]["launches"] += 1
                continue
            side = private_stream("timer")
            side.wait_stream(cur)
            graph = torch.cuda.CUDAGraph()
            try:
                with torch.cuda.stream(side):
                    fn()
                    graph.capture_begin(capture_error_mode=capture_error_mode())
                    for _ in range(reps):
                        fn()
                    graph.capture_end()
            except RuntimeError:
                graph = None
            cur.wait_stream(side)
            e0, e1 = torch.cuda.Event(enable_timing=True), torch.cuda.Event(enable_timing=True)
            e0.record()
            if graph is not None:
                graph.replay()
            else:
                for _ in range(reps):
                    fn()
            e1.record()
            e1.synchronize()
            res[key] = dict(name=name, launches=1, flop=fl, bytes=nb, ms=e0.elapsed_time(e1) / reps)
            del graph
        return res


timer = LaunchTimer()


def _pool_flops(scenes, bn):
    import numpy as np
    sz = np.diff(scenes.host_off).astype(np.float64)
    return float((sz * sz).sum()) * 512.0 * (4 + 2 * bn)


def _pool_flops_bn(scenes, bn):
    import numpy as np
    sz = np.diff(scenes.host_off).astype(np.float64)
    return float((sz * sz).sum()) * 512.0 * (4 * ((bn + 63) // 64) + 2 * bn)


def _pool_kname(bn, gpw, nchunks, bf16, dev, max_n=None, max_rows=None):
    if bf16:
        g = 4 if gpw >= 4 and bn <= 48 else (2 if gpw >= 2 else 1)
        if max_n is not None and max_n >= 32 and os.environ.get("SGG_POOL_JB") != "0":
            gj = "*" if max_rows is None else (4 if max_rows > 16 else (2 if max_rows > 8 else 1))
            return "sgg::pool_fwd_bf16_jb_kernel<%d, %s>" % (bn, gj)
        return "sgg::pool_fwd_bf16_kernel<%d, %d>" % (bn, g)
    if gpw <= 2 and 32 <= bn <= 48 and os.environ.get("SGG_POOL_X3", "1")[:1] != "0":
        return "sgg::pool_fwd_x3_kernel<%d, %d>" % (bn, gpw)
    small = gpw <= 2 and nchunks <= 4 * torch.cuda.get_device_properties(dev).multi_processor_count
    return "sgg::" + ("pool_fwd_v_kernel<%d, %d>" % (bn, gpw) if small else "pool_fwd_kernel<%d, %d, 2>" % (bn, gpw))


def _pool_wbytes(bn):
    return 4.0 * (1024 + bn * 512 + bn)


class PoolRider:

    def __init__(self):
        self.held = None
        self.done = False
        self.carried = False

    def hold(self, batch, keep, weights, bn, bf16, gpw, nchunks, work, launch):
        self.held = (batch, keep, weights, bn, bf16, gpw, nchunks, work, launch)

    def fits(self, weights, bn, bf16, gpw, wide=False):
        if self.held is None or wide:
            return False
        _, _, wh, bnh, bfh, gph, _, _, _ = self.held
        return bnh == bn and bfh == bf16 and gph == gpw and all(a is b for a, b in zip(wh, weights))

    def carry(self, batch, keep, nchunks, work):
        a, keep_a, (A, W2, b2), bn, bf16, gpw, nch_a, work_a, _ = self.held
        self.held = None
        self.done = self.carried = True
        lib = _lib()
        b = batch

        def pl(k=(keep_a, keep, A, W2, b2)):
            N.check(lib.sgg_pool_fwd2(N.ctypes.byref(a), N.ctypes.byref(b), N.ptr(A), N.ptr(W2), N.ptr(b2), bn,
                                      int(bf16), N.stream_ptr()), "sgg_pool_fwd2")
        S2, B2 = work_a[0] + work[0], work_a[1] + work[1]
        return pl, (None, S2, B2, work_a[2] + work[2], work_a[3] + work[3], nch_a + nchunks)

    def flush(self):
        if self.held is not None:
            _, _, (A, W2, b2), bn, bf16, gpw, nch, work, launch = self.held
            self.held = None
            launch()
            if timer.active:
                timer.add(_pool_kname(bn, gpw, nch, bf16, A.device), work[:2], work[2], work[3] + _pool_wbytes(bn),
                          launch)
        self.done = True


_PRIDER = [None]


def pool_pair():
    return _scoped(_PRIDER, PoolRider())


POOL_MAX_BN = 64
POOL_BN_MAX = 1024


def pool_bn_built(bn):
    from .scene import POOL_BUILT_BN
    return bn in POOL_BUILT_BN


def pool_is_wide(scenes):
    from .scene import SGG_POOL_MAX_PEDS, SGG_POOL_WIDE_MAX_PEDS
    if scenes.max_n > SGG_POOL_WIDE_MAX_PEDS:
        raise ValueError("social pooling: a scene of %d pedestrians exceeds the bound of %d per scene "
                         "(SGG_POOL_WIDE_MAX_PEDS)" % (scenes.max_n, SGG_POOL_WIDE_MAX_PEDS))
    return scenes.max_n > SGG_POOL_MAX_PEDS


def _pool_bn_bound(bn):
    if bn > POOL_BN_MAX:
        raise N.NativeError("social pooling: bottleneck_dim=%d exceeds the pooling kernels' bound of %d "
                            "(SGG_POOL_BN_MAX)" % (bn, POOL_BN_MAX))


def _pool_operands(h, pos, W1, We, be, b1, W2, b2, scenes, U=None, plan=None, prec=None):
    h = _rows(h, "h")
    pos = _req(pos, "pos").contiguous()
    B, Hd = h.shape
    E = We.shape[0]
    bn = W2.shape[0]
    assert pos.shape == (B, 2) and scenes.B == B, (pos.shape, B, scenes.B)
    assert W1.shape == (512, E + Hd), (W1.shape, E, Hd)
    _pool_bn_bound(bn)
    if plan is not None:
        plan = plan(scenes, bn, False)
    W1, W2, b2 = W1.contiguous(), W2.contiguous(), b2.contiguous()
    A, c = fold_fwd(W1[:, :E], We, be, b1)
    if U is None:
        U = xw_raw(h, W1[:, E:], c, trans_w=True, prec=prec)
    else:
        assert U.shape == (B, 512) and U.is_contiguous()
    out = torch.empty(B, bn, device=h.device, dtype=torch.float32)
    am = torch.empty(B, bn, device=h.device, dtype=torch.int32)
    return h, pos, W1, W2, b2, A, U, out, am, plan
# ... 2611 lines not shown
```

### group-gan-gcn-gat_amd/sgan/train_step.py

```python
import contextlib
import collections
import functools
import os
import random
import time

import numpy as np
import torch
import torch.distributed as dist

from . import kernels as K
from .models import get_noise
from .scene import SceneIndex


PAIR = os.environ.get("SGG_PAIR", "1") != "0"
DEC_PAIR = os.environ.get("SGG_DEC_PAIR", "1") != "0"


class TrainArgs:

    def __init__(self, **kw):
        self.obs_len = 8
        self.pred_len = 12
        self.best_k = 20
        self.l2_loss_weight = 1.0
        self.clipping_threshold_g = 2.0
        self.clipping_threshold_d = 0.0
        self.g_learning_rate = 1e-4
        self.d_learning_rate = 1e-3
        self.__dict__.update(kw)


def _sse_of(sc):
    return torch.from_numpy(np.stack([sc.host_off[:-1], sc.host_off[1:]], 1))


def _valid(sc):
    nv = getattr(sc, "nvalid", None)
    return {"nvalid": nv} if nv is not None else {}


class DataParallel:

    def __init__(self, group=None, exercise=False, capture=None, transport=None):
        self.on = dist.is_available() and dist.is_initialized()
        self.group = group
        self.world = dist.get_world_size(group) if self.on else 1
        self.rank = dist.get_rank(group) if self.on else 0
        self.exercise = bool(exercise) and self.on
        if transport is None:
            transport = os.environ.get("SGG_DP_TRANSPORT") or (
                "rccl" if self.on and "nccl" in str(dist.get_backend(group)) else "pg")
        if transport not in ("rccl", "pg"):
            raise ValueError("DataParallel: transport %r (rccl | pg)" % (transport,))
        self.transport = transport
        if capture is None:
            capture = transport == "rccl" and os.environ.get("SGG_CAPTURE_COLLECTIVE", "1") != "0"
        if capture and transport != "rccl":
            raise ValueError("DataParallel: only the rccl transport's all-reduce can be captured in a graph")
        self.capture = bool(capture) and self.on
        self.cut = None

    @property
    def rccl(self):
        if self.transport != "rccl" or not self.collective:
            return None
        from .rccl import comm_for
        return comm_for(self.group)

    def prepare(self):
        self.rccl

    @property
    def collective(self):
        return self.on and (self.world > 1 or self.exercise)

    @property
    def segmented(self):
        return self.collective and not self.capture

    def shard(self, S_global):
        if S_global < self.world:
            raise ValueError("scene-sharded DP needs >= %d scenes (one per rank), got %d: the reference loader "
                             "keeps a short last batch (loader.py:22-27); drop it or run it on fewer ranks"
                             % (self.world, S_global))
        per, rem = divmod(S_global, self.world)
        s0 = self.rank * per + min(self.rank, rem)
        return s0, s0 + per + (1 if self.rank < rem else 0)

    def allreduce_(self, tensors):
        if not self.collective or not tensors:
            return
        if self.cut is not None:
            self.cut(tensors)
            return
        flat = torch.cat([t.reshape(-1) for t in tensors])
        if self.transport == "rccl":
            self.rccl.allreduce_sum_(flat)
        else:
            dist.all_reduce(flat, op=dist.ReduceOp.SUM, group=self.group)
        views = flat.split([t.numel() for t in tensors])
        torch._foreach_copy_(tensors, [v.view_as(t) for v, t in zip(views, tensors)])


class StepInputs:

    def __init__(self, z_d, z_g, y):
        self.z_d, self.z_g, self.y = z_d, z_g, y


class KernelOps:
    traj_cat = staticmethod(K.traj_cat)
    l2_select = staticmethod(K.l2_select)
    l2_loss = staticmethod(K.l2_loss)
    bce_pair = staticmethod(K.bce_pair)
    bce_pair_total = staticmethod(K.bce_pair_total)
    split2 = staticmethod(K.split2)
    prefold = staticmethod(K.prefold)
    one = staticmethod(lambda device: K.const(1.0, device))
    optimizer = staticmethod(lambda params, lr: K.ClipAdam(params, lr=lr))
    handoff = staticmethod(K.bce_handoff)
    defer_finish = staticmethod(K.defer_grad_finish)
    shared_prefix = staticmethod(K.shared_prefix)
    traj_ahead = staticmethod(K.traj_ahead)
    decoder_pair = staticmethod(K.decoder_pair)
    glue_ride = staticmethod(K.glue_ride)
    eager_losses = staticmethod(K.eager_losses)


class GanTrainer:
    def __init__(self, G, D, args=None, dp=None, selective_backward=True, capturable=False, bce_pair=None, ops=None):
        self.G, self.D = G, D
        self.ops = ops or KernelOps()
        self._bce_override = bce_pair
        self.bce_pair = bce_pair or self.ops.bce_pair
        self.args = args or TrainArgs()
        self.dp = dp or DataParallel()
        self.selective_backward = selective_backward
        bn = [n for n, m in list(G.named_modules()) + list(D.named_modules()) if isinstance(m, torch.nn.BatchNorm1d)]
        if bn:
            raise NotImplementedError("GanTrainer: BatchNorm layers (%s) are not supported (train.py's batch_norm=0 "
                                      "default); drive the modules with the reference's own step functions" % bn[:3])
        gm = getattr(G, "gatencoder", None)
        gat = getattr(gm, "gat_intra", None) or getattr(gm, "gat_net", None)
        p1 = getattr(gat, "dropout", 0)
        if p1 and p1 > 0:
            raise NotImplementedError("GanTrainer: a generator with dropout1=%g is not supported (the shared G "
                                      "context would give all best_k samples one dropout mask); drive the modules "
                                      "with the reference's own step functions (scripts/train.py --dropout1)" % p1)
        pd = [m.dropout for m in (getattr(G, "pool_net", None), getattr(getattr(G, "decoder", None), "pool_net", None))
              if m is not None and getattr(m, "dropout", 0) and m.dropout > 0]
        if pd:
            raise NotImplementedError("GanTrainer: a generator whose pooling net has dropout=%g is not supported (the "
                                      "shared G context would give all best_k samples one dropout mask); drive the "
                                      "modules with the reference's own step functions (scripts/train.py --dropout)"
                                      % pd[0])
        self.g_params = list(G.parameters())
        self.d_params = list(D.parameters())
        self.opt_g = self.ops.optimizer(self.g_params, self.args.g_learning_rate)
        self.opt_d = self.ops.optimizer(self.d_params, self.args.d_learning_rate)

    def _noise(self, S_global, s0, s1):
        G = self.G
        if not G.noise_dim:
            return None
        if G.noise_mix_type != "global":
            raise NotImplementedError("GanTrainer shards scenes; per-ped noise ('ped' mix) is not sharded yet")
        z = get_noise((S_global,) + tuple(G.noise_dim), G.noise_type)
        return z[s0:s1]

    def _finish(self, params, opt, loss_terms, clip):
        K.pooldh_check()
        K.grad_flush()
        grads = [p.grad for p in params if p.grad is not None]
        if self.dp.collective:
            vals = torch.stack([t.detach().reshape(()) for t in loss_terms])
            self.dp.allreduce_(grads + [vals])
        else:
            vals = [t.detach().reshape(()) for t in loss_terms]
        opt.step(max_norm=clip)
        return vals

    def _prefix(self, obs_rel, copies):
        sp = getattr(self.ops, "shared_prefix", None)
        if sp is None or getattr(self.D, "encoder", None) is None or os.environ.get("SGG_NO_SHARED_PREFIX"):
            return contextlib.nullcontext()
        return sp(self.D, obs_rel, self.args.obs_len + self.args.pred_len, copies)

    def _traj_ahead(self, head, T1, ncol, col0=0, b=None, pos0=None):
        ta = getattr(self.ops, "traj_ahead", None)
        if ta is None:
            return contextlib.nullcontext()
        return ta(head, T1, ncol, col0, b, pos0)

    def _scope(self):
        st = contextlib.ExitStack()
        st.enter_context(getattr(self.ops, "handoff", contextlib.nullcontext)())
        if not self._grad_observed():
            st.enter_context(getattr(self.ops, "defer_finish", contextlib.nullcontext)())
        st.enter_context(getattr(self.ops, "glue_ride", contextlib.nullcontext)())
        return st

    def _grad_observed(self):
        for p in self.g_params + self.d_params:
            if getattr(p, "_backward_hooks", None) or getattr(p, "_post_accumulate_grad_hooks", None) \
                    or p.retains_grad:
                return True
        return False

    def d_step(self, batch, sc, S_global=None, B_global=None, shard=(0, None), inputs=None, pair=None):
        with self._scope():
            return self._d_step(batch, sc, S_global, B_global, shard, inputs, pair)

    def _pairs(self, sc, sc_g):
        G = self.G
        return (PAIR and self.selective_backward and self.args.best_k > 1 and self.args.l2_loss_weight > 0
                and hasattr(G, "context_pair") and G.pair_ok(sc, sc_g))

    def _d_step(self, batch, sc, S_global, B_global, shard, inputs, pair=None):
        a = self.args
        G = self.G
        (obs, pred_gt, obs_rel, pred_gt_rel, _ov, _pv, obs_g, _pg, _nl, _lm, sse) = batch
        g_kw = (S_global, B_global)
        S_global = S_global or sc.S
        B_global = B_global or sc.B
        s0 = shard[0]
        z = inputs.z_d if inputs is not None else self._noise(S_global, s0, s0 + sc.S)
        prefold = getattr(self.ops, "prefold", None)
        if prefold is not None and hasattr(G, "fold_specs") and hasattr(self.D, "fold_specs") \
                and G.num_layers == 1 and self.D.encoder.num_layers == 1:
            prefold(G.fold_specs() + self.D.fold_specs())
        pre = None
        dpair = getattr(self.ops, "decoder_pair", None)
        dpair = dpair() if (pair is not None and DEC_PAIR and dpair is not None) else contextlib.nullcontext()
        with self._prefix(obs_rel, 2):
            with dpair:
                with self._traj_ahead(obs_rel, pred_gt_rel.shape[0], sc.B, 0, pred_gt_rel, obs[0]):
                    if pair is not None:
                        bg, scg = pair
                        ctx_d, ctx_g = G.context_pair((obs, obs_rel, sse, obs_g, sc),
                                                      (bg[0], bg[2], bg[10], bg[6], scg))
                        with torch.no_grad():
                            fake_rel = G.decode(ctx_d, obs, obs_rel, sse, user_noise=z, scenes=sc)
                    else:
                        with torch.no_grad():
                            fake_rel = G(obs, obs_rel, sse, obs_g, user_noise=z, scenes=sc)
                    traj_rel, start = self.ops.traj_cat(obs_rel, fake_rel, pred_gt_rel, obs[0])
                if pair is not None:
                    self._no_shared = True
                    try:
                        pre = self._g_prefix(bg, scg, g_kw[0], g_kw[1], shard, inputs, ctx=ctx_g)
                    finally:
                        self._no_shared = False
            sc2 = sc.repeat(2)
            scores = self.D(start, traj_rel, _sse_of(sc2), scenes=sc2)
        if inputs is not None:
            y_real = inputs.y[0]
        else:
            y_real = random.uniform(0.7, 1.2)
            random.uniform(0, 0.3)
        loss = self.bce_pair(scores, sc.B, 0.0, y_real, sc.B / B_global, **_valid(sc))
        self.opt_d.zero_grad(set_to_none=True)
        torch.autograd.backward(loss, grad_tensors=self.ops.one(loss.device))
        vals = self._finish(self.d_params, self.opt_d, [loss], a.clipping_threshold_d)
        out = {"D_data_loss": vals[0], "D_total_loss": vals[0]}
        return out if pair is None else (out, pre)

    def g_step(self, batch, sc, S_global=None, B_global=None, shard=(0, None), inputs=None):
        with self._scope():
            return self._g_step(batch, sc, S_global, B_global, shard, inputs)

    def _g_step(self, batch, sc, S_global, B_global, shard, inputs):
        return self._g_rest(self._g_prefix(batch, sc, S_global, B_global, shard, inputs))

    def g_prefix(self, batch, sc, S_global=None, B_global=None, shard=(0, None), inputs=None, shared=False):
        if shared:
            return self._g_prefix(batch, sc, S_global, B_global, shard, inputs)
        self._no_shared = True
        try:
            return self._g_prefix(batch, sc, S_global, B_global, shard, inputs)
        finally:
            self._no_shared = False

    def g_rest(self, pre):
        with self._scope():
            return self._g_rest(pre)

    def _g_prefix(self, batch, sc, S_global, B_global, shard, inputs, ctx=None):
        a = self.args
        G, ops = self.G, self.ops
        (obs, pred_gt, obs_rel, pred_gt_rel, _ov, _pv, obs_g, _pg, _nl, loss_mask, sse) = batch
        S_global = S_global or sc.S
        B_global = B_global or sc.B
        s0 = shard[0]
        S, B, k = sc.S, sc.B, a.best_k
        mask = loss_mask[:, a.obs_len:]
        if inputs is not None:
            z_all = inputs.z_g
        else:
            zs = [self._noise(S_global, s0, s0 + S) for _ in range(k)]
            z_all = torch.stack(zs, 0) if zs[0] is not None else None
        use_l2 = a.l2_loss_weight > 0
        pfx = None if getattr(self, "_no_shared", False) else self._prefix(obs_rel, 1)
        if pfx is not None:
            pfx.__enter__()
        try:
            if ctx is None:
                ctx = G.context(obs, obs_rel, sse, obs_g, scenes=sc)
            best = None
            if self.selective_backward and k > 1 and use_l2:
                with torch.no_grad():
                    pred_all = G.decode(ctx.detach(), obs, obs_rel, sse, user_noise=z_all, scenes=sc, copies=k,
                                        noise_index=(None, 0))
                    best = ops.l2_select(pred_all, pred_gt_rel, mask, sc, k)
        except BaseException:
            if pfx is not None:
                pfx.__exit__(None, None, None)
            raise
        return dict(batch=batch, sc=sc, S_global=S_global, B_global=B_global, z_all=z_all, ctx=ctx, best=best,
                    pfx=pfx, mask=mask, inputs=inputs)

    def _g_rest(self, pre):
        a = self.args
        G, D, ops = self.G, self.D, self.ops
        batch, sc, B_global, z_all, ctx, pfx, mask, inputs = (pre[n] for n in (
            "batch", "sc", "B_global", "z_all", "ctx", "pfx", "mask", "inputs"))
        (obs, pred_gt, obs_rel, pred_gt_rel, _ov, _pv, obs_g, _pg, _nl, loss_mask, sse) = batch
        with contextlib.ExitStack() as stack:
            S, B, k = sc.S, sc.B, a.best_k
            use_l2 = a.l2_loss_weight > 0
            if pfx is None:
                stack.enter_context(self._prefix(obs_rel, 1))
            else:
                stack.push(pfx)
            if self.selective_backward and k > 1:
                best = pre["best"]
                copies = 2 if use_l2 else 1
                tah = self._traj_ahead(obs_rel, a.pred_len, B, (copies - 1) * B)
                tah.__enter__()
                try:
                    out = G.decode(ctx, obs, obs_rel, sse, user_noise=z_all, scenes=sc, copies=copies,
                                   noise_index=(best, k - 1))
                except BaseException:
                    tah.__exit__(None, None, None)
                    raise
                if use_l2:
                    fake_rel_best, fake_rel_last = ops.split2(out, B)
                else:
                    fake_rel_best, fake_rel_last = None, out
            else:
                tah = contextlib.nullcontext()
                out = G.decode(ctx, obs, obs_rel, sse, user_noise=z_all, scenes=sc, copies=k, noise_index=(None, 0))
                fake_rel_last = out[:, (k - 1) * B:]
                fake_rel_best = None
                if use_l2:
                    seg = sc.ped_scene_long()
                    m = mask.t().unsqueeze(2)
                    l2s = torch.stack([(m * (pred_gt_rel - out[:, i * B:(i + 1) * B]) ** 2).sum((0, 2))
                                       for i in range(k)], 0)
                    scene_l2 = torch.zeros(k, S, device=obs.device).index_add_(1, seg, l2s)
                    mask_sum = torch.zeros(S, device=obs.device).index_add_(0, seg, mask.sum(1))
            terms = []
            total = getattr(self.ops, "bce_pair_total", None)
            fused_total = use_l2 and total is not None and self._bce_override is None
            eager = contextlib.nullcontext if fused_total else getattr(self.ops, "eager_losses", contextlib.nullcontext)
            if use_l2:
                if fake_rel_best is not None:
                    with eager():
                        g_l2 = ops.l2_loss(fake_rel_best, pred_gt_rel, mask, sc, a.l2_loss_weight)
                else:
                    g_l2 = (a.l2_loss_weight * scene_l2.min(0)[0] / mask_sum).sum()
                terms.append(g_l2)
            for p in self.d_params:
                p.requires_grad_(False)
            try:
                scores = D(obs[:1], ops.traj_cat(obs_rel, fake_rel_last), sse, scenes=sc)
            finally:
                tah.__exit__(None, None, None)
                stack.close()
                for p in self.d_params:
                    p.requires_grad_(True)
            y = inputs.y[2] if inputs is not None else random.uniform(0.7, 1.2)
            if terms and fused_total:
                adv, loss = total(scores, scores.shape[0], y, y, sc.B / B_global, terms[0], **_valid(sc))
            else:
                with eager():
                    adv = self.bce_pair(scores, scores.shape[0], y, y, sc.B / B_global, **_valid(sc))
                loss = adv + (terms[0] if terms else 0.0)
            self.opt_g.zero_grad(set_to_none=True)
            torch.autograd.backward(loss, grad_tensors=self.ops.one(loss.device), inputs=self._g_inputs())
            vals = self._finish(self.g_params, self.opt_g, [terms[0] if terms else adv * 0, adv, loss],
                                a.clipping_threshold_g)
            out = {"G_discriminator_loss": vals[1], "G_total_loss": vals[2]}
            if use_l2:
                out["G_l2_loss_rel"] = vals[0]
            return out

    def _g_inputs(self):
        if not hasattr(self, "_g_in"):
            graph = getattr(self.G, "graph", "gat")
            skip = {"gat": ("gcn_module.",), "gcn": ("gatencoder.", "mlp_decoder_context."),
                    "sgangat": ("mlp_decoder_context.",), "vanilla": ()}.get(graph, ())
            self._g_in = [p for n, p in self.G.named_parameters() if not n.startswith(skip)]
        return self._g_in

    def step(self, batch, sc, batch_g=None, sc_g=None, **kw):
        bg, scg = (batch, sc) if batch_g is None else (batch_g, sc_g)
        if self._pairs(sc, scg):
            ld, pre = self.d_step(batch, sc, pair=(bg, scg), **kw)
            return ld, self.g_rest(pre)
        ld = self.d_step(batch, sc, **kw)
        lg = self.g_step(bg, scg, **kw)
        return ld, lg

    def step_split(self, batch, sc, batch_g=None, sc_g=None, **kw):
        if kw.get("inputs") is None and self.G.noise_dim:
            raise ValueError("step_split: pass inputs=StepInputs (draw_inputs) -- the G-step's noise is used first")
        pre = self.g_prefix(batch if batch_g is None else batch_g, sc if sc_g is None else sc_g, **kw)
        ld = self.d_step(batch, sc, **kw)
        lg = self.g_rest(pre)
        return ld, lg

    def draw_inputs(self, S_global, s0, s1):
        z_d = self._noise(S_global, s0, s1)
        yr, yf = random.uniform(0.7, 1.2), random.uniform(0, 0.3)
        z_g = [self._noise(S_global, s0, s1) for _ in range(self.args.best_k)]
        yg = random.uniform(0.7, 1.2)
        zg = torch.stack(z_g, 0) if z_g[0] is not None else None
        return z_d, zg, torch.tensor([yr, yf, yg], dtype=torch.float32)


class DrawSource:

    def __init__(self, draw):
        self.draw = draw
        self.pending = collections.deque()
        self.seq = 0

    def ahead(self, n):
        while len(self.pending) < n:
            self.pending.append(self.draw())
        return self.seq, [self.pending[j] for j in range(n)]

    def pop(self, n):
        for _ in range(n):
            self.pending.popleft()
        self.seq += n

    def take(self):
        self.ahead(1)
        item = self.pending[0]
        self.pop(1)
        return item


class GraphedTrainer:

    def __init__(self, trainer, batch, sc, S_global=None, B_global=None, shard=(0, None), warmup=2, batch_g=None,
                 sc_g=None, draw=None, prologue=None, iters=1, overlap=False, draw_ahead=False, draws=None,
                 head=None):
        self.t = trainer
        self.ar_events = None
        self.iters = iters = max(1, int(iters))
        self.overlap = overlap = bool(overlap) and not trainer.dp.collective
        self.prologue = prologue or (lambda: None)
        self.head = head
        self.batch, self.sc = batch, sc
        self.batch_g, self.sc_g = batch_g, sc_g
        if batch_g is not None:
            assert sc_g is not None and (sc_g.S, sc_g.B) == (sc.S, sc.B), "G-step batch must match the D-step's sizes"
        self.kw = dict(S_global=S_global or sc.S, B_global=B_global or sc.B, shard=shard)
        dev = batch[0].device
        s0 = shard[0]
        self.span = (self.kw["S_global"], s0, s0 + sc.S)
        self.draws = draws if draws is not None else DrawSource(
            draw or functools.partial(trainer.draw_inputs, *self.span))
        self.draw = self.draws.take
        G = trainer.G
        nd = tuple(G.noise_dim) if G.noise_dim else None
        k = trainer.args.best_k
        shp = [(sc.S,) + (nd or ()), (k, sc.S) + (nd or ()), (3,)] if nd else [(3,)]
        sizes = [int(np.prod(x)) for x in shp]
        per = sum(sizes)
# ... 381 lines not shown
```

### include/sgg.h

```cpp
#ifndef SGG_H
#define SGG_H

#include <stdint.h>
#include <stddef.h>

#ifdef __cplusplus
extern "C" {
#endif

#define SGG_E_ARG (-1)

int sgg_version(void);
const char* sgg_last_error(void);
const char* sgg_source_hash(void);

#define SGG_POOL_MAX_PEDS 64
#define SGG_POOL_BN_MAX 1024
#define SGG_POOL_WIDE_MAX_PEDS 1024
#define SGG_GAT_MAX_NODES 128
#define SGG_GAT_WIDE_MAX_NODES 1024

int sgg_xw(const float* X, int ldx, const float* Xmask, int ldm, const float* W, int ldw, int trans_w,
           const float* bias, float* Y, int ldy, int M, int K, int N, int act, void* stream);

int sgg_xw_bf16(const float* X, int ldx, const float* Xmask, int ldm, const float* W, int ldw, int trans_w,
                const float* bias, float* Y, int ldy, int M, int K, int N, int act, void* stream);

int sgg_pool_plan(const int32_t* host_scene_off, int S, int bn, int target_chunks, int max_gpw,
                  int32_t* host_chunks, int cap, int* max_rows, int* gpw);
int sgg_pool_fwd(const float* U, const float* pos, const float* A, const float* W2,
                 const float* b2, const int32_t* scene_off, const int32_t* chunks, int nchunks,
                 int max_rows, int gpw, int B, int bn, int max_n, float* out, int32_t* argmax,
                 const int32_t* nchunks_dev, void* stream);

int sgg_pool_plan_bf16(const int32_t* host_scene_off, int S, int bn, int target_chunks, int32_t* host_chunks,
                       int cap, int* max_rows, int* gpw);
int sgg_pool_fwd_bf16(const float* U, const float* pos, const float* A, const float* W2,
                      const float* b2, const int32_t* scene_off, const int32_t* chunks, int nchunks,
                      int max_rows, int gpw, int B, int bn, int max_n, float* out, int32_t* argmax,
                      const int32_t* nchunks_dev, void* stream);

typedef struct SggPoolBatch {
  const float* U;
  const float* pos;
  const int32_t* scene_off;
  const int32_t* chunks;
  int nchunks;
  int max_rows;
  int gpw;
  int B;
  int max_n;
  float* out;
  int32_t* argmax;
  const int32_t* nchunks_dev;
} SggPoolBatch;
int sgg_pool_fwd2(const SggPoolBatch* a, const SggPoolBatch* b, const float* A, const float* W2, const float* b2,
                  int bn, int bf16, void* stream);

int sgg_pool_dh_dw(const float* dU, int ldu, const float* W, int ldw, float* dh, int ldh, int accumulate,
                   const float* h, int ldx, int B, int H, float* ws, size_t ws_bytes, void* stream);

int sgg_pool_bwd_grid(int S);
int sgg_pool_bwd(const float* U, const float* pos, const float* A, const float* W2,
                 const float* out, const int32_t* argmax, const float* dout,
                 const int32_t* scene_off, int S, int B, int bn, int max_n,
                 float* dU, float* part, void* stream);

int sgg_pool_plan_wide(const int32_t* host_scene_off, int S, int bn, int target_chunks, int32_t* host_chunks,
                       int cap, int* max_rows, int* gpw);
int sgg_pool_fwd_wide(const float* U, const float* pos, const float* A, const float* W2,
                      const float* b2, const int32_t* scene_off, const int32_t* chunks, int nchunks,
                      int max_rows, int gpw, int B, int bn, int max_n, float* out, int32_t* argmax,
                      void* stream);
int sgg_pool_bwd_wide_grid(int S, int max_n);
int sgg_pool_bwd_wide(const float* U, const float* pos, const float* A, const float* W2,
                      const float* out, const int32_t* argmax, const float* dout,
                      const int32_t* scene_off, int S, int B, int bn, int max_n,
                      float* dU, float* part, void* stream);

int sgg_pool_plan_bn(const int32_t* host_scene_off, int S, int bn, int target_chunks, int32_t* host_chunks,
                     int cap, int* max_rows, int* gpw);
int sgg_pool_fwd_bn(const float* U, const float* pos, const float* A, const float* W2,
                    const float* b2, const int32_t* scene_off, const int32_t* chunks, int nchunks,
                    int max_rows, int gpw, int B, int bn, int max_n, float* out, int32_t* argmax,
                    void* stream);
int sgg_pool_bwd_bn_grid(int S, int bn, int max_n);
long long sgg_pool_bwd_bn_ws_floats(int S, int B, int bn, int max_n);
int sgg_pool_bwd_bn(const float* U, const float* pos, const float* A, const float* W2,
                    const float* out, const int32_t* argmax, const float* dout,
                    const int32_t* scene_off, int S, int B, int bn, int max_n,
                    float* dU, float* part, size_t part_floats, void* stream);

int sgg_gat_fwd(const float* Wh, int heads, const float* a, const float* bias, const float* labels,
                const int32_t* seg_off, int nseg, int n, int F, float alpha, int mask_mode,
                int epilogue, int max_seg, float* hp, float* y, int ldy, void* stream);

int sgg_gat_bwd(const float* Wh, int heads, const float* a, const float* labels, const int32_t* seg_off,
                int nseg, int n, int F, float alpha, int mask_mode, int epilogue, int max_seg,
                const float* hp, const float* y, const float* dy, int lddy,
                float* dWh, float* ds, float* dt, void* stream);

int sgg_gat_fwd_ex(const float* Wh, int heads, const float* a_src, const float* a_dst, const float* bias,
                   const float* labels, const int32_t* seg_off, int nseg, int n, int F, float alpha, int mask_mode,
                   int epilogue, int max_seg, float* hp, float* y, int ldy, void* stream);

size_t sgg_gat_bwd_ex_work_bytes(int nseg, int heads, int F);
int sgg_gat_bwd_ex(const float* Wh, int heads, const float* a_src, const float* a_dst, const float* labels,
                   const int32_t* seg_off, int nseg, int n, int F, float alpha, int mask_mode, int epilogue,
                   int max_seg, const float* hp, const float* y, const float* dy, int lddy, float* dWh,
                   float* da_src, float* da_dst, float* dbias, void* work, void* stream);

size_t sgg_gat_wide_work_floats(int n, int nseg, int heads, int F, int max_seg);
int sgg_gat_fwd_wide(const float* Wh, int heads, const float* a_src, const float* a_dst, int lda,
                     const float* bias, const float* labels, const int32_t* seg_off, int nseg, int n, int F,
                     float alpha, int mask_mode, int epilogue, int max_seg, float* hp, float* y, int ldy,
                     float* work, void* stream);
int sgg_gat_bwd_wide(const float* Wh, int heads, const float* a_src, const float* a_dst, int lda,
                     const float* labels, const int32_t* seg_off, int nseg, int n, int F, float alpha,
                     int mask_mode, int epilogue, int max_seg, const float* hp, const float* y,
                     const float* dy, int lddy, float* dWh, float* ds, float* dt, float* da_src,
                     float* da_dst, float* dbias, float* work, void* stream);

int sgg_gat_fwd_drop(const float* Wh, int heads, const float* a_src, const float* a_dst, int lda,
                     const float* bias, const float* labels, const int32_t* seg_off, int nseg, int n, int F,
                     float alpha, int mask_mode, int epilogue, int max_seg, float* hp, float* y, int ldy,
                     float p, unsigned long long seed, unsigned offset, unsigned site, unsigned head0,
                     const unsigned long long* rng_dev, void* stream);
int sgg_gat_bwd_drop(const float* Wh, int heads, const float* a_src, const float* a_dst, int lda,
                     const float* labels, const int32_t* seg_off, int nseg, int n, int F, float alpha,
                     int mask_mode, int epilogue, int max_seg, const float* hp, const float* y,
                     const float* dy, int lddy, float* dWh, float* ds, float* dt, float* da_src,
                     float* da_dst, float* dbias, void* work, float p, unsigned long long seed,
                     unsigned offset, unsigned site, unsigned head0, const unsigned long long* rng_dev,
                     void* stream);
int sgg_dropout(const float* x, int ldx, int rows, int cols, float p, unsigned long long seed, unsigned offset,
                unsigned site, const unsigned long long* rng_dev, float* y, int ldy, void* stream);

size_t sgg_gat_layer_lds_bytes(int K, int F, int max_seg);
int sgg_gat_layer_fwd(const float* x1, int ld1, int K1, const float* x2, int ld2, int K2, const float* w,
                      const float* a_src, const float* a_dst, const float* bias, const int32_t* seg_off, int nseg,
                      int n, int heads, int F, float alpha, float eps, int epilogue, int max_seg, int bf16,
                      float* xn, float* rstd, float* wh, float* hp, float* y, int ldy, void* stream);

typedef struct SggGatLayerSet {
  const float* x1;
  int ld1, K1;
  const float* x2;
  int ld2, K2;
  const int32_t* seg_off;
  int nseg, n, max_seg;
  float *xn, *rstd, *wh, *hp, *y;
  int ldy;
} SggGatLayerSet;
int sgg_gat_layer_fwd2(const SggGatLayerSet* a, const SggGatLayerSet* b, const float* w, const float* a_src,
                       const float* a_dst, const float* bias, int heads, int F, float alpha, float eps,
                       int epilogue, int bf16, void* stream);

int sgg_seg_norm_fwd(const float* x, int ldx, int F, const int32_t* seg_off, int nseg, float eps,
                     float* y, int ldy, float* rstd, void* stream);

int sgg_seg_norm_bwd(const float* y, int ldy, const float* dy, int lddy, int F, const int32_t* seg_off,
                     int nseg, const float* rstd, float* dx, int lddx, void* stream);

size_t sgg_group_index_ws(int S, int B);
int sgg_group_index(const float* labels, const int32_t* scene_off, int S, int B, int max_n,
                    int32_t* ped_gid, int32_t* ped_scene, int32_t* group_off,
                    int32_t* group_scene, int32_t* group_count, void* workspace, void* stream);

int sgg_seg_reduce(const float* x, int ldx, int F, const int32_t* seg_of_row,
                   const float* row_scale, const int32_t* range_off, const int32_t* seg_range,
                   const int32_t* nseg_dev, int nseg_cap, int mean, float* out, int ldo,
                   void* stream);

int sgg_seg_gather(const float* src, int lds, int F, const int32_t* seg_of_row,
                   const float* row_scale, const int32_t* nrow_dev, int n, float* out, int ldo,
                   void* stream);

int sgg_xtw_splits(int R, int M, int N);
int sgg_xtw(const float* X, int ldx, const float* Y, int ldy, const float* Ymask, int ldm, int R, int M, int N,
            float* C, int ldc, int trans_c, float* colsum, float* ws, size_t ws_bytes, void* stream);
int sgg_xtw_partial(const float* X, int ldx, const float* Y, int ldy, const float* Ymask, int ldm, int R, int M,
                    int N, int colsum, float* ws, size_t ws_bytes, void* stream);

#define SGG_RED_MAX 24
#define SGG_FOLDB_MAX 6
typedef struct {
  const float* src;
  int rows;
  int ld;
  int col0;
  int cols;
  float* out;
  int map;
  int N;
  int ldo;
  int trans;
} SggRed;
typedef struct {
  const float* W;
  int ldw;
  int R;
  int E;
  const float* We;
  const float* be;
  const float* dA_src;
  int dA_rows;
  int dA_ld;
  int dA_col0;
  const float* db_src;
  int db_rows;
  int db_ld;
  int db_col0;
  float* dW;
  int lddw;
  float* dWe;
  float* dbe;
  float* dbias_copy;
} SggFoldBwd;
int sgg_grad_finish(const SggRed* reds, int nred, const SggFoldBwd* folds, int nfold, float* scratch,
                    size_t scratch_bytes, void* stream);

#define SGG_LOSSJOB_MAX 2
typedef struct {
  const float* term;
  int S;
  float* loss;
} SggL2Job;
typedef struct {
  const float* x;
  int n;
  int split;
  const float* ya;
  const float* yb;
  float w;
  float* loss;
  const float* addend;
  float* total;
  const int32_t* nvalid;
} SggBceJob;
int sgg_grad_finish_losses(const SggRed* reds, int nred, const SggFoldBwd* folds, int nfold, float* scratch,
                           size_t scratch_bytes, const SggL2Job* l2, int nl2, const SggBceJob* bce, int nbce,
                           void* stream);

int sgg_head_ok(int K, int N1);
int sgg_head_slab_cols(int K, int N1);
int sgg_head_fwd(const float* X, int ldx, int M, int K, int N1, const float* W1, const float* b1, const float* w2,
                 const float* b2, int act, float* hid, float* Y, void* stream);
int sgg_head_bwd(const float* X, int ldx, int M, int K, int N1, const float* W1, const float* w2, const float* hid,
                 const float* Y, const float* dY, int act, float* dX, int lddx, float* wslab, const float* bce_g,
                 const float* bce_ya, const float* bce_yb, int bce_split, float bce_w, const int32_t* bce_nvalid,
                 void* stream);
int sgg_head_fwdbwd(const float* X, int ldx, int M, int K, int N1, const float* W1, const float* b1, const float* w2,
                    const float* b2, int act, float* Y, float* dX, int lddx, float* wslab, const float* bce_g,
                    const float* bce_ya, const float* bce_yb, int bce_split, float bce_w, const int32_t* bce_nvalid,
                    void* stream);

int sgg_fold_fwd(const float* W, int ldw, int R, int E, const float* We, const float* be,
                 const float* b1, const float* b2, float* A, float* bias, void* stream);
#define SGG_FOLD_MAX 8
typedef struct {
  const float* W;
  int ldw;
  int R;
  int E;
  const float* We;
  const float* be;
  const float* b1;
  const float* b2;
  float* A;
  float* bias;
} SggFold;
int sgg_fold_fwd_multi(const SggFold* folds, int n, void* stream);
int sgg_fold_bwd(const float* W, int ldw, int R, int E, const float* We, const float* be, const float* dA,
                 const float* dbias, float* dW, int lddw, float* dWe, float* dbe, float* dbias_copy, void* stream);

long long sgg_lstm_state_floats(int T, int B, int H, int which);
long long sgg_lstm_dg_floats(int T, int B, int H);
int sgg_lstm_fwd(const float* rel, const float* A, const float* Whh, const float* bias,
                 const float* h0, const float* c0, const float* Wp, const float* bp, int T, int B, int H,
                 int decoder, float* h_all, float* c_all, float* act_all, float* rel_out,
                 void* stream);
typedef struct {
  const float* ctx;
  int ldc;
  int Dc;
  const float* z;
  int nz;
  const int64_t* best;
  int first_k;
  const int32_t* ped_scene;
  int S;
  int Bper;
  const float* last_rel;
} SggDecInit;
typedef struct {
  float* out;
  int NB;
  int T0;
  int col0;
  int ncol;
  const float* head;
  int ldh;
  const float* b;
  int ldb;
  const float* pos0;
  float* start;
} SggTrajOut;
int sgg_lstm_fwd_dec(const SggDecInit* di, const float* A, const float* Whh, const float* bias, const float* Wp,
                     const float* bp, int T, int B, int H, float* h_all, float* c_all, float* act_all,
                     float* rel_out, float* rel0_out, const SggTrajOut* to, void* stream);
int sgg_lstm_fwd_dec2(const SggDecInit* di, const SggDecInit* di2, const float* A, const float* Whh,
                      const float* bias, const float* Wp, const float* bp, int T, int B, int B2, int H,
                      float* rel_out, float* rel_out2, const SggTrajOut* to2, void* stream);

int sgg_lstm_u_ok(int T, int B, int H, int decoder, int save, int NU);
int sgg_lstm_fwd_u(const float* rel, const float* A, const float* Whh, const float* bias, const float* h0,
                   const float* c0, int T, int B, int H, float* h_all, float* c_all, float* act_all,
                   const float* Wu, int ldwu, const float* cu, int NU, float* U, void* stream);

int sgg_lstm_wpart_rows(int H, int B);
const char* sgg_lstm_kernel_name(int H, int B, int decoder, int save, int bwd);
int sgg_lstm_bwd_split(const float* A, const float* Whh, const float* Wp, const float* h_all, const float* c_all,
                       const float* act_all, const float* rel, const float* rel_out, const float* dout,
                       const float* dout2, int bsplit, int T, int B, int H, float* dh0, float* drel_in,
                       float* drel_tot, float* wpart, void* stream);
int sgg_lstm_bwd_tail(const float* A, const float* Whh, const float* h_all, const float* c_all,
                      const float* act_all, const float* rel, const float* dh_last, int T, int B, int H,
                      int t_stop, float* drel_in, void* stream);
int sgg_lstm_bwd(const float* A, const float* Whh, const float* Wp, const float* h_all, const float* c_all,
                 const float* act_all, const float* rel, const float* rel_out, const float* dh_last,
                 const float* dout, int T, int B, int H, int decoder, float* dG, float* dh0,
                 float* drel_in, float* drel_tot, float* wpart, void* stream);

typedef struct {
  const float* rel;
  const float* A;
  const float* Whh;
  const float* bias;
  const float* h0;
  const float* c0;
  int T, B, Bl, t0, Tl, Bsrc;
  float* h_all;
  float* c_all;
  float* act_all;
  const float* Wu;
  int ldwu;
  const float* cu;
  int NU;
  float* U;
} SggLstmSeg;
int sgg_lstm_fwd_seg(const SggLstmSeg* seg, int H, void* stream);
int sgg_lstm_fwd_seg2(const SggLstmSeg* a, int Ha, const SggLstmSeg* b, int Hb, void* stream);
int sgg_lstm_fwd_seg3(const SggLstmSeg* a, int Ha, const SggLstmSeg* b, int Hb, const SggLstmSeg* c, int Hc,
                      void* stream);
int sgg_lstm_fwd_dec_seg(const SggDecInit* di, const float* A, const float* Whh, const float* bias, const float* Wp,
                         const float* bp, int T, int B, int H, float* h_all, float* c_all, float* act_all,
                         float* rel_out, float* rel0_out, const SggTrajOut* to, const SggLstmSeg* pre, int Hp,
                         void* stream);
int sgg_lstm_bwd_shared(const float* A, const float* Whh, const float* h_all, const float* c_all,
                        const float* act_all, const float* rel, const float* dh_last, int T, int B, int H,
                        int t_sh, int Bsrc, float* drel_in, float* wpart, void* stream);

typedef struct {
  const float* dU;
  int ldu;
  const float* W1h;
  int ldw;
  const float* base;
  int NU;
  const float* h;
  int ldh;
  float* ws;
  size_t ws_bytes;
  int splits;
} SggPoolDh;
int sgg_lstm_bwd_pooldh_ok(int H);
int sgg_lstm_bwd_pooldh_pays(int B, int H);
int sgg_lstm_bwd_pooldh_rides(int B, int H, int NU);
int sgg_lstm_bwd_pooldh(const float* A, const float* Whh, const float* h_all, const float* c_all,
                        const float* act_all, const float* rel, const SggPoolDh* src, int T, int B, int H, int t_stop,
                        int t_sh, int Bsrc, float* dh0, float* drel_in, float* wpart, void* stream);

int sgg_bce_fwd(const float* x, int n, int split, const float* ya, const float* yb, float w, float* loss,
                const float* addend, float* total, const int32_t* nvalid, void* stream);

int sgg_bce_bwd(const float* x, int n, int split, const float* ya, const float* yb, float w,
                const float* gout, float* dx, const int32_t* nvalid, void* stream);

int sgg_adam_parts(long long total);
int sgg_adam_step(float* const* params, float* const* grads, float* const* exp_avg, float* const* exp_avg_sq,
                  const long long* numel, int n, double lr, double beta1, double beta2, float eps, float max_norm,
                  float* const* step, float* ws, size_t ws_bytes, void* stream);

#define SGG_GATENC_MAX_HEADS 4
typedef struct {
  const float* Wi[SGG_GATENC_MAX_HEADS];
  const float* ai[SGG_GATENC_MAX_HEADS];
  const float* Wio;
  const float* aio;
  const float* Wg[SGG_GATENC_MAX_HEADS];
  const float* ag[SGG_GATENC_MAX_HEADS];
  const float* Wgo;
  const float* ago;
  const float* Woe;
  const float* boe;
} SggGatEncWeights;

typedef struct {
  const float* X;
  int ldx;
  const float* labels;
  const int32_t* scene_off;
  int S;
  int np;
  int nh;
  float alpha;
  SggGatEncWeights w;
  float* y;
  int ldy;
  const float* dy;
  int lddy;
  float* dX;
  int lddx;
  float* slab;
  float* saved;
  const float* X2;
  int ldx2;
  int kx1;
  float* dX2;
  int lddx2;
  int dy_copies;
  int dy_cstride;
} SggGatEncArgs;

int sgg_gatenc_param_size(int nh);
long long sgg_gatenc_saved_floats(int S, int max_n, int nh);
long long sgg_gatenc_lds_bytes(int max_n, int nh, int bwd);
int sgg_gatenc_fwd(const SggGatEncArgs* args, void* stream);
int sgg_gatenc_fwd2(const SggGatEncArgs* a, const SggGatEncArgs* b, void* stream);
int sgg_gatenc_bwd(const SggGatEncArgs* args, void* stream);

typedef struct {
  const float* X;
  int ldx;
  const float* X2;
  int ldx2;
  int kx1;
  const float* labels;
  const int32_t* scene_off;
  int S;
  int np;
  int fin;
  int fe;
  int bf16;
  const float* W0i;
  const float* W1i;
  const float* W0g;
  const float* W1g;
  const float* Woe;
  const float* boe;
  float* y;
  int ldy;
  const float* dy;
  int lddy;
  int dy_copies;
  int dy_cstride;
  float* dX;
  int lddx;
  float* dX2;
  int lddx2;
  float* slab;
} SggGcnModArgs;

int sgg_gcnmod_param_size(int fin, int fe);
int sgg_gcnmod_slab_rows(int S);
long long sgg_gcnmod_lds_bytes(int max_n, int fin, int fe, int bwd);
int sgg_gcnmod_fwd(const SggGcnModArgs* args, void* stream);
int sgg_gcnmod_fwd2(const SggGcnModArgs* a, const SggGcnModArgs* b, void* stream);
int sgg_gcnmod_bwd(const SggGcnModArgs* args, void* stream);

int sgg_slab_reduce(const float* slab, int rows, int cols, float* out, void* stream);

int sgg_traj_cat(const float* head, int ldh, int T0, const float* a, int lda, const float* b, int ldb, int T1, int B,
                 float* out, const float* pos0, float* start, void* stream);

int sgg_decoder_init(const float* ctx, int ldc, int Dc, const float* z, int nz, const int64_t* best, int first_k,
                     int copies, const int32_t* ped_scene, int S, int B, const float* last_rel, float* h0,
                     float* rel0, void* stream);

int sgg_l2_select(const float* pred, const float* gt, const float* mask, int ldm, const int32_t* scene_off, int S,
                  int T, int B, int k, int64_t* best, void* stream);

int sgg_l2_loss_fwd(const float* pred, int ldp, const float* gt, const float* mask, int ldm, const int32_t* scene_off,
                    int S, int T, int B, float w, float* loss, float* msum, float* term_ws, void* stream);
int sgg_l2_loss_bwd(const float* pred, int ldp, const float* gt, const float* mask, int ldm, const int32_t* ped_scene,
                    const float* msum, int T, int B, float w, const float* gout, float* dpred, int ldd, void* stream);
int sgg_l2_loss_bwd_scenes(const float* pred, int ldp, const float* gt, const float* mask, int ldm,
                           const int32_t* scene_off, int S, int T, int B, float w, const float* gout, float* dpred,
                           int ldd, float* term, void* stream);

#define SGG_GLUE_NONE 0
#define SGG_GLUE_SELECT 1
#define SGG_GLUE_L2BWD 2
typedef struct {
  int kind;
  const float* pred;
  int ldp;
  const float* gt;
  const float* mask;
  int ldm;
  const int32_t* scene_off;
  int S, T, B, k;
  int64_t* best;
  float w;
  const float* gout;
  float* dpred;
  int ldd;
  float* term;
} SggGlueSeg;
int sgg_lstm_fwd_seg_glue(const SggLstmSeg* seg, int H, const SggGlueSeg* glue, void* stream);

long long sgg_gather_batch_floats(int B, int obs_len, int pred_len);
int sgg_gather_batch(const float* table, int rec, const int32_t* rows, int B, int obs_len, int pred_len, float* out,
                     void* stream);

#define SGG_VAL_SLOTS 11
size_t sgg_val_metrics_work_floats(int B);
int sgg_val_metrics(const float* pred_rel, const float* gt, const float* gt_rel, const float* start,
                    const float* mask, int ld, const float* non_linear, const float* scores, float y_real, int T,
                    int B, double* acc, float* work, void* stream);

typedef struct SggDecStep {
  int B, H, bn, mlp_dim, NU, mlp, cell, ldwu;
  const float *h_prev, *pool_prev, *c_prev, *r_in, *pos_prev;
  const float *W1m, *b1m, *W2m, *b2m, *A, *Whh, *bias, *Wp, *bp, *Wu, *cu;
  float *h, *c, *rel, *pos, *U;
  float *act, *h_mix, *z1;
} SggDecStep;
typedef struct SggDecStepBwd {
  int B, H, bn, mlp_dim, mlp, cell;
  const float *dh, *dc, *drel, *dpos;
  const float *act, *c, *c_prev, *h_mix, *z1;
  const float *W1m, *W2m, *A, *Whh, *Wp;
  float *dh_prev, *dpool_prev, *dc_prev, *dr_in, *dpos_prev;
  float *dG, *dz2, *dz1, *drel_tot;
} SggDecStepBwd;
int sgg_dec_step_ok(int H, int bn, int mlp_dim, int NU);
long long sgg_dec_step_saved_floats(int B, int H, int mlp_dim);
int sgg_dec_step_fwd(const SggDecStep* a, void* stream);
int sgg_dec_step_bwd(const SggDecStepBwd* a, void* stream);

int sgg_pool_dpos(const float* U, const float* pos, const float* A, const float* W2, const float* out,
                  const int32_t* argmax, const float* dout, const int32_t* scene_off, int S, int B, int bn,
                  float* dpos, void* stream);

#define SGG_POOL_DROP_SITE_HIDDEN 16
#define SGG_POOL_DROP_SITE_OUT 17
int sgg_pool_fwd_bn_drop(const float* U, const float* pos, const float* A, const float* W2,
                         const float* b2, const int32_t* scene_off, const int32_t* chunks, int nchunks,
                         int max_rows, int gpw, int B, int bn, int max_n, float* out, int32_t* argmax,
                         float p, unsigned long long seed, unsigned offset,
                         const unsigned long long* rng_dev, void* stream);
int sgg_pool_bwd_bn_drop(const float* U, const float* pos, const float* A, const float* W2,
                         const float* out, const int32_t* argmax, const float* dout,
                         const int32_t* scene_off, int S, int B, int bn, int max_n,
                         float* dU, float* part, size_t part_floats, float p, unsigned long long seed,
                         unsigned offset, const unsigned long long* rng_dev, void* stream);
int sgg_pool_dpos_drop(const float* U, const float* pos, const float* A, const float* W2, const float* out,
                       const int32_t* argmax, const float* dout, const int32_t* scene_off, int S, int B, int bn,
                       float* dpos, float p, unsigned long long seed, unsigned offset,
                       const unsigned long long* rng_dev, void* stream);

#define SGG_POOL_NORM_MAX_PEDS 256
#define SGG_POOL_NORM_FIN_ROWS 32
int sgg_pool_norm_fwd(const float* U, const float* pos, const float* A, const float* gamma1,
                      const float* beta1, const float* W2, const float* b2, const float* gamma2,
                      const float* beta2, const int32_t* scene_off, int S, int B, int bn, int min_n,
                      int max_n, float eps1, float eps2, float* Un, float* An, float* mu1, float* var1,
                      float* mu2, float* var2, float* out, int32_t* argmax, void* stream);
int sgg_pool_norm_running(const float* mean, const float* var, const int32_t* scene_off, int S, int C,
                          float momentum, float* running_mean, float* running_var, void* stream);
int sgg_pool_norm_bwd_rows(int bn);
long long sgg_pool_norm_bwd_ws_floats(int S, int B, int bn);
long long sgg_pool_norm_bwd_slab_offset(int S, int B);
int sgg_pool_norm_bwd(const float* U, const float* pos, const float* A, const float* gamma1,
                      const float* W2, const float* b2, const float* gamma2, const float* beta2,
                      const float* Un, const float* An, const float* mu1, const float* var1,
                      const float* mu2, const float* var2, const float* out, const int32_t* argmax,
                      const float* dout, const int32_t* scene_off, int S, int B, int bn, int min_n,
                      int max_n, float eps1, float eps2, int wgrad, float* dU, float* dpos, float* ws,
                      size_t ws_floats, void* stream);

#ifdef __cplusplus
}
#endif
#endif
```

Baseline: 145,200 scenes/s.

## Fuse fold backward and refolding of folded weights into the Adam update kernel

The Adam update kernel gains extra workgroups, one per folded layer (W, We, be, b1, b2). Each of these optionally computes the fold backward (dW, dWe, dbe from dA and dbias), applies Adam to the fold operands, and recomputes the folded A and bias from the updated parameters. The flat path skips those tensors via per-tensor skip/ld masks. This removes the separate fold backward launch and the later fold forward recomputation, at the cost of a 1024-thread block with large LDS use and a more complex kernel and planning path on the host.

```diff
diff --git a/group-gan-gcn-gat_amd/csrc/adam.hip b/group-gan-gcn-gat_amd/csrc/adam.hip
--- a/group-gan-gcn-gat_amd/csrc/adam.hip
+++ b/group-gan-gcn-gat_amd/csrc/adam.hip
@@ -1,4 +1,5 @@
 #include "sgg_common.h"
+#include "adam_fold_body.h"
 
 namespace sgg {
 
@@ -13,13 +14,25 @@
   float* v[kAdamMaxTensors];
   float* step[kAdamMaxTensors];
   long long off[kAdamMaxTensors + 1];
+  int skip[kAdamMaxTensors];
+  int ld[kAdamMaxTensors];
   int n;
 };
+
+struct AdamFolds {
+  SggAdamFold f[SGG_FOLD_MAX];
+  int n;
+};
+static_assert(sizeof(AdamList) + sizeof(AdamFolds) + 128 <= 4096, "adam_update_kernel: kernel arguments over 4 KB");
+
+constexpr int kFoldMaxE = 64;
+constexpr int kFoldMaxR = 512;
+constexpr int kFoldLds = kFoldMaxR * 17;
 
 __device__ __forceinline__ float block_sum(float x, float* red) {
   for (int o = 32; o > 0; o >>= 1) x += __shfl_xor(x, o);
   const int lane = threadIdx.x & 63, wave = threadIdx.x >> 6;
-  if (lane == 0) red[wave] = x;
+  if (lane == 0 && wave < kAdamThreads / 64) red[wave] = x;
   __syncthreads();
   float s = 0.f;
 #pragma unroll
@@ -33,11 +46,12 @@
 struct Tab {
   long long lo, hi;
   unsigned long long p, g, m, v;
+  int skip, ld;
 };
 
 __device__ __forceinline__ Tab lane_tab(const AdamList& L) {
   const int t = threadIdx.x & 63;
-  Tab r = {0, 0, 0, 0, 0, 0};
+  Tab r = {0, 0, 0, 0, 0, 0, 0, 1};
   if (t < L.n) {
     r.lo = L.off[t];
     r.hi = L.off[t + 1];
@@ -45,6 +59,8 @@
     r.g = reinterpret_cast<unsigned long long>(L.g[t]);
     r.m = reinterpret_cast<unsigned long long>(L.m[t]);
     r.v = reinterpret_cast<unsigned long long>(L.v[t]);
+    r.skip = L.skip[t];
+    r.ld = L.ld[t];
   }
   return r;
 }
@@ -114,7 +130,237 @@
   if (threadIdx.x == 0) partial[blockIdx.x] = s;
 }
 
-__global__ void __launch_bounds__(kAdamThreads) adam_update_kernel(AdamList L, int nparts, float max_norm,
+__device__ __forceinline__ void step_scalars(bool fused, float lss, float lbc, const float* __restrict__ scal, int k,
+                                             float& ss, float& bc) {
+  if (fused) {
+    ss = __shfl(lss, k);
+    bc = __shfl(lbc, k);
+  } else {
+    ss = scal[2 * k];
+    bc = scal[2 * k + 1];
+  }
+}
+
+__device__ __forceinline__ void adam_flat_wg(const AdamList& L, const Tab& T, bool clip, float coef, float beta2,
+                                             float w1, float w2, float eps, bool fused, float lss, float lbc,
+                                             const float* __restrict__ scal) {
+  const long long e0 = (long long)blockIdx.x * kAdamChunk;
+  int ek[kAdamPer];
+  long long ei[kAdamPer];
+  chunk_elems(L, T, e0, ek, ei);
+  float* pp[kAdamPer];
+  float* gp[kAdamPer];
+  float* mp[kAdamPer];
+  float* vp[kAdamPer];
+  float gr[kAdamPer], m0[kAdamPer], v0[kAdamPer], p0[kAdamPer], ss[kAdamPer], bc[kAdamPer];
+#pragma unroll
+  for (int u = 0; u < kAdamPer; ++u) {
+    const int k = ek[u] >= 0 ? ek[u] : 0;
+    const long long i = ek[u] >= 0 ? ei[u] : 0;
+    pp[u] = reinterpret_cast<float*>(shfl64(T.p, k)) + i;
+    gp[u] = reinterpret_cast<float*>(shfl64(T.g, k)) + i;
+    mp[u] = reinterpret_cast<float*>(shfl64(T.m, k)) + i;
+    vp[u] = reinterpret_cast<float*>(shfl64(T.v, k)) + i;
+    step_scalars(fused, lss, lbc, scal, k, ss[u], bc[u]);
+    const int sk = __shfl(T.skip, k), ld = __shfl(T.ld, k);
+    if (sk > 0 && (int)((unsigned)i % (unsigned)ld) < sk) ek[u] = -1;
+  }
+#pragma unroll
+  for (int u = 0; u < kAdamPer; ++u) {
+    gr[u] = *gp[u];
+    m0[u] = *mp[u];
+    v0[u] = *vp[u];
+    p0[u] = *pp[u];
+  }
+#pragma unroll
+  for (int u = 0; u < kAdamPer; ++u) {
+    if (ek[u] < 0) continue;
+    float g = gr[u];
+    if (clip) {
+      g = clip_scale(g, coef);
+      *gp[u] = g;
+    }
+    float mi, vi, pi;
+    adam_elem(g, m0[u], v0[u], p0[u], w1, w2, beta2, ss[u], bc[u], eps, mi, vi, pi);
+    *mp[u] = mi;
+    *vp[u] = vi;
+    *pp[u] = pi;
+  }
+}
+
+constexpr int kFoldThreads = 1024;
+constexpr int kFoldRowsPer = (kFoldMaxR + kFoldThreads - 1) / kFoldThreads;
+constexpr int kFoldPer = 4;
+
+__device__ __forceinline__ void adam_fold_wg(const AdamList& L, const SggAdamFold& d, bool clip, float coef,
+                                             float beta2, float w1, float w2, float eps, const float (&ss)[5],
+                                             const float (&bc)[5]) {
+  __shared__ float g3[3 * kFoldMaxR];
+  __shared__ float part[3 * 512];
+  __shared__ float sW[kFoldLds];
+  __shared__ float sWe[2 * kFoldMaxE];
+  __shared__ float sbe[kFoldMaxE];
+  const int t = threadIdx.x, R = d.R, E = d.E, ldw = d.ldw;
+  float* const Wp = L.p[d.W];
+  float* const Wg = L.g[d.W];
+  float* const Wm = L.m[d.W];
+  float* const Wv = L.v[d.W];
+  if (d.dA) {
+    for (int r = t; r < R; r += kFoldThreads) {
+      const float2 a = reinterpret_cast<const float2*>(d.dA)[r];
+      const float b = d.dbias[r];
+      g3[3 * r] = a.x;
+      g3[3 * r + 1] = a.y;
+      g3[3 * r + 2] = b;
+      if (d.dbias_copy) d.dbias_copy[r] = b;
+    }
+    __syncthreads();
+    const float* We = L.p[d.We];
+    const float* be = L.p[d.be];
+    const int ng = 512 / E;
+    for (int vt = t; vt < ng * E; vt += kFoldThreads) {
+      const int e = vt % E, g = vt / E;
+      const float we0 = We[2 * e], we1 = We[2 * e + 1], bee = be[e];
+      float s0 = 0.f, s1 = 0.f, s2 = 0.f;
+#pragma unroll 8
+      for (int r = g; r < R; r += ng) {
+        const float a0 = g3[3 * r], a1 = g3[3 * r + 1], b = g3[3 * r + 2];
+        Wg[(size_t)r * ldw + e] = fold_dw_term(a0, a1, b, we0, we1, bee);
+        const float w = Wp[(size_t)r * ldw + e];
+        s0 = fmaf(w, a0, s0);
+        s1 = fmaf(w, a1, s1);
+        s2 = fmaf(w, b, s2);
+      }
+      part[3 * vt] = s0;
+      part[3 * vt + 1] = s1;
+      part[3 * vt + 2] = s2;
+    }
+    __syncthreads();
+    if (t < 3 * E) {
+      const int e = t / 3, j = t - 3 * e;
+      float s = 0.f;
+      for (int g = 0; g < ng; ++g) s += part[3 * (g * E + e) + j];
+      if (j < 2) L.g[d.We][2 * e + j] = s;
+      else L.g[d.be][e] = s;
+    }
+    __syncthreads();
+  }
+  const bool ina = t < 3 * E;
+  const int aw = t < 2 * E;
+  const int ai = ina ? (aw ? t : t - 2 * E) : 0, ak = aw ? d.We : d.be;
+  float* const agp = L.g[ak] + ai;
+  float* const amp = L.m[ak] + ai;
+  float* const avp = L.v[ak] + ai;
+  float* const app = L.p[ak] + ai;
+  const float ag = *agp, am = *amp, av = *avp, ap = *app;
+  const bool has2 = d.b2 >= 0;
+  const int k2 = has2 ? d.b2 : d.b1;
+  float bg[2][kFoldRowsPer], bm[2][kFoldRowsPer], bv[2][kFoldRowsPer], bp[2][kFoldRowsPer];
+  int br[kFoldRowsPer];
+#pragma unroll
+  for (int j = 0; j < kFoldRowsPer; ++j) {
+    const int r = t + j * kFoldThreads;
+    br[j] = r < R ? r : 0;
+    bg[0][j] = L.g[d.b1][br[j]];
+    bm[0][j] = L.m[d.b1][br[j]];
+    bv[0][j] = L.v[d.b1][br[j]];
+    bp[0][j] = L.p[d.b1][br[j]];
+    bg[1][j] = L.g[k2][br[j]];
+    bm[1][j] = L.m[k2][br[j]];
+    bv[1][j] = L.v[k2][br[j]];
+    bp[1][j] = L.p[k2][br[j]];
+  }
+  if (ina) {
+    float gi = ag;
+    if (clip) {
+      gi = clip_scale(gi, coef);
+      *agp = gi;
+    }
+    float mi, vi, pi;
+    adam_elem(gi, am, av, ap, w1, w2, beta2, aw ? ss[1] : ss[2], aw ? bc[1] : bc[2], eps, mi, vi, pi);
+    *amp = mi;
+    *avp = vi;
+    *app = pi;
+    if (aw) sWe[ai] = pi;
+    else sbe[ai] = pi;
+  }
+  float nb[2][kFoldRowsPer];
+#pragma unroll
+  for (int j = 0; j < kFoldRowsPer; ++j) {
+    nb[0][j] = nb[1][j] = 0.f;
+    if (t + j * kFoldThreads >= R) continue;
+#pragma unroll
+    for (int q = 0; q < 2; ++q) {
+      if (q == 1 && !has2) continue;
+      const int k = q ? k2 : d.b1;
+      float gi = bg[q][j];
+      if (clip) {
+        gi = clip_scale(gi, coef);
+        L.g[k][br[j]] = gi;
+      }
+      float mi, vi, pi;
+      adam_elem(gi, bm[q][j], bv[q][j], bp[q][j], w1, w2, beta2, q ? ss[4] : ss[3], q ? bc[4] : bc[3], eps, mi, vi,
+                pi);
+      L.m[k][br[j]] = mi;
+      L.v[k][br[j]] = vi;
+      L.p[k][br[j]] = pi;
+      nb[q][j] = pi;
+    }
+  }
+  const int nW = R * E;
+  for (int i0 = 0; i0 < nW; i0 += kFoldThreads * kFoldPer) {
+    int off[kFoldPer], lo[kFoldPer];
+    bool ok[kFoldPer];
+    float g[kFoldPer], m0[kFoldPer], v0[kFoldPer], p0[kFoldPer];
+#pragma unroll
+    for (int u = 0; u < kFoldPer; ++u) {
+      const int idx = i0 + t + u * kFoldThreads;
+      ok[u] = idx < nW;
+      const int r = ok[u] ? idx / E : 0, e = ok[u] ? idx - r * E : 0;
+      off[u] = r * ldw + e;
+      lo[u] = r * (E + 1) + e;
+    }
+#pragma unroll
+    for (int u = 0; u < kFoldPer; ++u) {
+      g[u] = Wg[off[u]];
+      m0[u] = Wm[off[u]];
+      v0[u] = Wv[off[u]];
+      p0[u] = Wp[off[u]];
+    }
+#pragma unroll
+    for (int u = 0; u < kFoldPer; ++u) {
+      if (!ok[u]) continue;
+      float gi = g[u];
+      if (clip) {
+        gi = clip_scale(gi, coef);
+        Wg[off[u]] = gi;
+      }
+      float mi, vi, pi;
+      adam_elem(gi, m0[u], v0[u], p0[u], w1, w2, beta2, ss[0], bc[0], eps, mi, vi, pi);
+      Wm[off[u]] = mi;
+      Wv[off[u]] = vi;
+      Wp[off[u]] = pi;
+      sW[lo[u]] = pi;
+    }
+  }
+  __syncthreads();
+#pragma unroll
+  for (int j = 0; j < kFoldRowsPer; ++j) {
+    const int r = t + j * kFoldThreads;
+    if (r >= R) continue;
+    float a0 = 0.f, a1 = 0.f, bb = 0.f;
+    const float* w = sW + r * (E + 1);
+#pragma unroll 8
+    for (int e = 0; e < E; ++e) fold_fwd_step(w[e], sWe[2 * e], sWe[2 * e + 1], sbe[e], a0, a1, bb);
+    d.A[2 * r] = a0;
+    d.A[2 * r + 1] = a1;
+    d.bias[r] = fold_bias(bb, nb[0][j], has2 ? nb[1][j] : 0.f);
+  }
+}
+
+template <int NT>
+__global__ void __launch_bounds__(NT) adam_update_kernel(AdamList L, AdamFolds F, int nparts,
+                                                                   float max_norm,
                                                                    const float* __restrict__ partial,
                                                                    const float* __restrict__ scal, float beta2,
                                                                    float w1, float w2, float eps,
@@ -122,7 +368,6 @@
                                                                    double beta1d, double beta2d) {
   __shared__ float red[kAdamThreads / 64];
   __shared__ int last;
-  const long long e0 = (long long)blockIdx.x * kAdamChunk;
   const Tab T = lane_tab(L);
   float tstep = 0.f, lss = 0.f, lbc = 1.f;
   if (ticket && (int)(threadIdx.x & 63) < L.n) {
@@ -130,57 +375,24 @@
     lss = (float)(lr / (1.0 - pow(beta1d, (double)tstep)));
     lbc = (float)sqrt(1.0 - pow(beta2d, (double)tstep));
   }
-  int ek[kAdamPer];
-  long long ei[kAdamPer];
-  chunk_elems(L, T, e0, ek, ei);
   float coef = 1.f;
   if (max_norm > 0.f) {
     float acc = 0.f;
-    for (int q = threadIdx.x; q < nparts; q += kAdamThreads) acc += partial[q];
+    if (threadIdx.x < kAdamThreads)
+      for (int q = threadIdx.x; q < nparts; q += kAdamThreads) acc += partial[q];
     const float norm = sqrtf(block_sum(acc, red));
     coef = fminf(max_norm / (norm + 1e-6f), 1.f);
   }
-  float* pp[kAdamPer];
-  float* gp[kAdamPer];
-  float* mp[kAdamPer];
-  float* vp[kAdamPer];
-  float gr[kAdamPer], m0[kAdamPer], v0[kAdamPer], p0[kAdamPer], ss[kAdamPer], bc[kAdamPer];
-#pragma unroll
-  for (int u = 0; u < kAdamPer; ++u) {
-    const int k = ek[u] >= 0 ? ek[u] : 0;
-    const long long i = ek[u] >= 0 ? ei[u] : 0;
-    pp[u] = reinterpret_cast<float*>(shfl64(T.p, k)) + i;
-    gp[u] = reinterpret_cast<float*>(shfl64(T.g, k)) + i;
-    mp[u] = reinterpret_cast<float*>(shfl64(T.m, k)) + i;
-    vp[u] = reinterpret_cast<float*>(shfl64(T.v, k)) + i;
-    if (ticket) {
-      ss[u] = __shfl(lss, k);
-      bc[u] = __shfl(lbc, k);
-    } else {
-      ss[u] = scal[2 * k];
-      bc[u] = scal[2 * k + 1];
-    }
-  }
-#pragma unroll
-  for (int u = 0; u < kAdamPer; ++u) {
-    gr[u] = *gp[u];
-    m0[u] = *mp[u];
-    v0[u] = *vp[u];
-    p0[u] = *pp[u];
-  }
-#pragma unroll
-  for (int u = 0; u < kAdamPer; ++u) {
-    if (ek[u] < 0) continue;
-    float g = gr[u];
-    if (max_norm > 0.f) {
-      g *= coef;
-      *gp[u] = g;
-    }
-    const float mi = m0[u] + w1 * (g - m0[u]);
-    const float vi = v0[u] * beta2 + w2 * g * g;
-    *mp[u] = mi;
-    *vp[u] = vi;
-    *pp[u] = p0[u] + -ss[u] * (mi / (sqrtf(vi) / bc[u] + eps));
+  if ((int)blockIdx.x >= nparts) {
+    const SggAdamFold& d = F.f[blockIdx.x - nparts];
+    const int ti[5] = {d.W, d.We, d.be, d.b1, d.b2};
+    float fss[5], fbc[5];
+#pragma unroll
+    for (int j = 0; j < 5; ++j)
+      step_scalars(ticket != nullptr, lss, lbc, scal, ti[j] < 0 ? 0 : ti[j], fss[j], fbc[j]);
+    adam_fold_wg(L, d, max_norm > 0.f, coef, beta2, w1, w2, eps, fss, fbc);
+  } else if (threadIdx.x < kAdamThreads) {
+    adam_flat_wg(L, T, max_norm > 0.f, coef, beta2, w1, w2, eps, ticket != nullptr, lss, lbc, scal);
   }
   if (ticket) {
     __syncthreads();
@@ -201,18 +413,24 @@
   return (int)((total + kAdamChunk - 1) / kAdamChunk) + 2 * kAdamMaxTensors + 1;
 }
 
-extern "C" int sgg_adam_step(float* const* params, float* const* grads, float* const* exp_avg,
-                             float* const* exp_avg_sq, const long long* numel, int n, double lr, double beta1,
-                             double beta2, float eps, float max_norm, float* const* step, float* ws,
-                             size_t ws_bytes, void* stream) {
-  SGG_CHECK_ARG(params && grads && exp_avg && exp_avg_sq && numel && step, "sgg_adam_step: null pointer");
-  SGG_CHECK_ARG(n >= 1 && n <= kAdamMaxTensors, "sgg_adam_step: %d tensors (1..%d)", n, kAdamMaxTensors);
+static int adam_step_impl(const char* who, float* const* params, float* const* grads, float* const* exp_avg,
+                          float* const* exp_avg_sq, const long long* numel, int n, double lr, double beta1,
+                          double beta2, float eps, float max_norm, float* const* step, float* ws, size_t ws_bytes,
+                          const SggAdamFold* folds, int nfolds, void* stream) {
+  SGG_CHECK_ARG(params && grads && exp_avg && exp_avg_sq && numel && step, "%s: null pointer", who);
+  SGG_CHECK_ARG(n >= 1 && n <= kAdamMaxTensors, "%s: %d tensors (1..%d)", who, n, kAdamMaxTensors);
+  SGG_CHECK_ARG(nfolds >= 0 && nfolds <= SGG_FOLD_MAX && (nfolds == 0 || folds), "%s: 0 <= nfolds <= %d (got %d)", who,
+                SGG_FOLD_MAX, nfolds);
   AdamList L;
   L.n = n;
   L.off[0] = 0;
+  for (int i = 0; i < kAdamMaxTensors; ++i) {
+    L.skip[i] = 0;
+    L.ld[i] = 1;
+  }
   for (int i = 0; i < n; ++i) {
-    SGG_CHECK_ARG(params[i] && grads[i] && exp_avg[i] && exp_avg_sq[i] && step[i] && numel[i] >= 0,
-                  "sgg_adam_step: tensor %d", i);
+    SGG_CHECK_ARG(params[i] && grads[i] && exp_avg[i] && exp_avg_sq[i] && step[i] && numel[i] >= 0, "%s: tensor %d",
+                  who, i);
     L.p[i] = params[i];
     L.g[i] = grads[i];
     L.m[i] = exp_avg[i];
@@ -220,11 +438,34 @@
     L.step[i] = step[i];
     L.off[i + 1] = L.off[i] + numel[i];
   }
+  const int clip = max_norm > 0.f;
+  AdamFolds F = {};
+  F.n = nfolds;
+  for (int k = 0; k < nfolds; ++k) {
+    const SggAdamFold& d = folds[k];
+    SGG_CHECK_ARG(d.E >= 1 && d.E <= kFoldMaxE && d.R >= 1 && d.R <= kFoldMaxR && d.ldw >= d.E &&
+                      (long long)d.R * (d.E + 1) <= kFoldLds,
+                  "%s: fold %d: bad sizes R=%d E=%d ldw=%d", who, k, d.R, d.E, d.ldw);
+    const int ti[5] = {d.W, d.We, d.be, d.b1, d.b2};
+    const long long want[5] = {(long long)d.R * d.ldw, 2LL * d.E, d.E, d.R, d.R};
+    for (int j = 0; j < 5; ++j) {
+      if (j == 4 && ti[j] == -1) continue;
+      SGG_CHECK_ARG(ti[j] >= 0 && ti[j] < n && numel[ti[j]] == want[j], "%s: fold %d: operand %d is not a tensor of %lld",
+                    who, k, j, want[j]);
+      SGG_CHECK_ARG(L.skip[ti[j]] == 0, "%s: fold %d: tensor %d belongs to two folds", who, k, ti[j]);
+      L.skip[ti[j]] = j == 0 ? d.E : (int)want[j];
+      L.ld[ti[j]] = j == 0 ? d.ldw : (int)want[j];
+    }
+    SGG_CHECK_ARG(d.A && d.bias, "%s: fold %d: null output", who, k);
+    SGG_CHECK_ARG((d.dA == nullptr) == (d.dbias == nullptr) && (d.dA || !d.dbias_copy) &&
+                      (reinterpret_cast<uintptr_t>(d.dA) & 7) == 0,
+                  "%s: fold %d: bad (dA, dbias)", who, k);
+    SGG_CHECK_ARG(!(d.dA && clip), "%s: fold %d: the fold backward rides only without clipping", who, k);
+    F.f[k] = d;
+  }
   const int parts = sgg_adam_parts(L.off[n]) - 2 * kAdamMaxTensors - 1;
   if (parts == 0) return 0;
-  const int clip = max_norm > 0.f;
-  SGG_CHECK_ARG(ws && ws_bytes >= sizeof(float) * ((size_t)parts + 2 * kAdamMaxTensors + 1),
-                "sgg_adam_step: workspace");
+  SGG_CHECK_ARG(ws && ws_bytes >= sizeof(float) * ((size_t)parts + 2 * kAdamMaxTensors + 1), "%s: workspace", who);
   hipStream_t st = (hipStream_t)stream;
   unsigned* ticket = reinterpret_cast<unsigned*>(ws);
   float* partial = ws + 1;
@@ -232,8 +473,29 @@
   if (clip)
     hipLaunchKernelGGL(adam_prep_kernel, dim3(parts), dim3(kAdamThreads), 0, st, L, clip, partial, scal, lr, beta1,
                        beta2);
-  hipLaunchKernelGGL(adam_update_kernel, dim3(parts), dim3(kAdamThreads), 0, st, L, parts, clip ? max_norm : 0.f,
-                     partial, scal, (float)beta2, (float)(1.0 - beta1), (float)(1.0 - beta2), eps, clip ? nullptr : ticket,
-                     lr, beta1, beta2);
-  SGG_RETURN_LAUNCH("sgg_adam_step");
-}
+  if (nfolds > 0)
+    hipLaunchKernelGGL(adam_update_kernel<kFoldThreads>, dim3(parts + nfolds), dim3(kFoldThreads), 0, st, L, F, parts,
+                       clip ? max_norm : 0.f, partial, scal, (float)beta2, (float)(1.0 - beta1), (float)(1.0 - beta2),
+                       eps, clip ? nullptr : ticket, lr, beta1, beta2);
+  else
+    hipLaunchKernelGGL(adam_update_kernel<kAdamThreads>, dim3(parts), dim3(kAdamThreads), 0, st, L, F, parts,
+                       clip ? max_norm : 0.f, partial, scal, (float)beta2, (float)(1.0 - beta1), (float)(1.0 - beta2),
+                       eps, clip ? nullptr : ticket, lr, beta1, beta2);
+  SGG_RETURN_LAUNCH(who);
+}
+
+extern "C" int sgg_adam_step(float* const* params, float* const* grads, float* const* exp_avg,
+                             float* const* exp_avg_sq, const long long* numel, int n, double lr, double beta1,
+                             double beta2, float eps, float max_norm, float* const* step, float* ws,
+                             size_t ws_bytes, void* stream) {
+  return adam_step_impl("sgg_adam_step", params, grads, exp_avg, exp_avg_sq, numel, n, lr, beta1, beta2, eps, max_norm,
+                        step, ws, ws_bytes, nullptr, 0, stream);
+}
+
+extern "C" int sgg_adam_step_folds(float* const* params, float* const* grads, float* const* exp_avg,
+                                   float* const* exp_avg_sq, const long long* numel, int n, double lr, double beta1,
+                                   double beta2, float eps, float max_norm, float* const* step, float* ws,
+                                   size_t ws_bytes, const SggAdamFold* folds, int nfolds, void* stream) {
+  return adam_step_impl("sgg_adam_step_folds", params, grads, exp_avg, exp_avg_sq, numel, n, lr, beta1, beta2, eps,
+                        max_norm, step, ws, ws_bytes, folds, nfolds, stream);
+}
diff --git a/group-gan-gcn-gat_amd/csrc/adam_fold_body.h b/group-gan-gcn-gat_amd/csrc/adam_fold_body.h
--- /dev/null
+++ b/group-gan-gcn-gat_amd/csrc/adam_fold_body.h
@@ -0,0 +1,37 @@
+#pragma once
+#include <hip/hip_runtime.h>
+
+namespace sgg {
+
+__device__ __forceinline__ void adam_elem(float g, float m0, float v0, float p0, float w1, float w2, float beta2,
+                                          float ss, float bc, float eps, float& mi, float& vi, float& pi) {
+#pragma clang fp contract(off)
+  mi = m0 + w1 * (g - m0);
+  vi = v0 * beta2 + (w2 * g) * g;
+  const float den = sqrtf(vi) / bc + eps;
+  pi = fmaf(-ss, mi / den, p0);
+}
+
+__device__ __forceinline__ float clip_scale(float g, float coef) {
+#pragma clang fp contract(off)
+  return g * coef;
+}
+
+__device__ __forceinline__ float fold_dw_term(float a0, float a1, float b, float we0, float we1, float bee) {
+#pragma clang fp contract(off)
+  return fmaf(a0, we0, fmaf(a1, we1, b * bee));
+}
+
+__device__ __forceinline__ void fold_fwd_step(float w, float we0, float we1, float bee, float& a0, float& a1,
+                                              float& bb) {
+  a0 = fmaf(w, we0, a0);
+  a1 = fmaf(w, we1, a1);
+  bb = fmaf(w, bee, bb);
+}
+
+__device__ __forceinline__ float fold_bias(float bb, float b1, float b2) {
+#pragma clang fp contract(off)
+  return bb + b1 + b2;
+}
+
+}
diff --git a/group-gan-gcn-gat_amd/csrc/fold.hip b/group-gan-gcn-gat_amd/csrc/fold.hip
--- a/group-gan-gcn-gat_amd/csrc/fold.hip
+++ b/group-gan-gcn-gat_amd/csrc/fold.hip
@@ -1,4 +1,5 @@
 #include "sgg_common.h"
+#include "adam_fold_body.h"
 
 namespace sgg {
 
@@ -11,14 +12,11 @@
     const float* w = W + (size_t)r * ldw;
 #pragma unroll 8
     for (int e = 0; e < E; ++e) {
-      const float we = w[e];
-      a0 = fmaf(we, We[2 * e], a0);
-      a1 = fmaf(we, We[2 * e + 1], a1);
-      bb = fmaf(we, be[e], bb);
+      fold_fwd_step(w[e], We[2 * e], We[2 * e + 1], be[e], a0, a1, bb);
     }
     A[2 * r] = a0;
     A[2 * r + 1] = a1;
-    bias[r] = bb + b1[r] + (b2 ? b2[r] : 0.f);
+    bias[r] = fold_bias(bb, b1[r], b2 ? b2[r] : 0.f);
   }
 }
 
@@ -33,14 +31,11 @@
     const float* w = d.W + (size_t)r * d.ldw;
 #pragma unroll 8
     for (int e = 0; e < d.E; ++e) {
-      const float we = w[e];
-      a0 = fmaf(we, d.We[2 * e], a0);
-      a1 = fmaf(we, d.We[2 * e + 1], a1);
-      bb = fmaf(we, d.be[e], bb);
+      fold_fwd_step(w[e], d.We[2 * e], d.We[2 * e + 1], d.be[e], a0, a1, bb);
     }
     d.A[2 * r] = a0;
     d.A[2 * r + 1] = a1;
-    d.bias[r] = bb + d.b1[r] + (d.b2 ? d.b2[r] : 0.f);
+    d.bias[r] = fold_bias(bb, d.b1[r], d.b2 ? d.b2[r] : 0.f);
   }
 }
 
@@ -69,7 +64,7 @@
 #pragma unroll 8
     for (int r = g; r < R; r += ng) {
       const float a0 = g3[3 * r], a1 = g3[3 * r + 1], b = g3[3 * r + 2];
-      dW[(size_t)r * lddw + e] = fmaf(a0, we0, fmaf(a1, we1, b * bee));
+      dW[(size_t)r * lddw + e] = fold_dw_term(a0, a1, b, we0, we1, bee);
       const float w = W[(size_t)r * ldw + e];
       s0 = fmaf(w, a0, s0);
       s1 = fmaf(w, a1, s1);
diff --git a/group-gan-gcn-gat_amd/csrc/grad.hip b/group-gan-gcn-gat_amd/csrc/grad.hip
--- a/group-gan-gcn-gat_amd/csrc/grad.hip
+++ b/group-gan-gcn-gat_amd/csrc/grad.hip
@@ -160,6 +160,13 @@
 extern "C" int sgg_grad_finish_losses(const SggRed* reds, int nred, const SggFoldBwd* folds, int nfold,
                                       float* scratch, size_t scratch_bytes, const SggL2Job* l2, int nl2,
                                       const SggBceJob* bce, int nbce, void* stream) {
+  return sgg_grad_finish_sums(reds, nred, folds, nfold, nfold, scratch, scratch_bytes, l2, nl2, bce, nbce, stream);
+}
+
+extern "C" int sgg_grad_finish_sums(const SggRed* reds, int nred, const SggFoldBwd* folds, int nfold, int nrun,
+                                    float* scratch, size_t scratch_bytes, const SggL2Job* l2, int nl2,
+                                    const SggBceJob* bce, int nbce, void* stream) {
+  SGG_CHECK_ARG(nrun >= 0 && nrun <= nfold, "sgg_grad_finish_sums: 0 <= nrun <= nfold (got %d, %d)", nrun, nfold);
   SGG_CHECK_ARG(nl2 >= 0 && nl2 <= SGG_LOSSJOB_MAX && nbce >= 0 && nbce <= SGG_LOSSJOB_MAX &&
                     (nl2 == 0 || l2) && (nbce == 0 || bce),
                 "sgg_grad_finish_losses: 0 <= nl2, nbce <= %d (got %d, %d)", SGG_LOSSJOB_MAX, nl2, nbce);
@@ -227,16 +234,16 @@
   if (nl2 + nbce > 0) ++blk;
   hipStream_t st = (hipStream_t)stream;
   if (blk > 0) hipLaunchKernelGGL(grad_finish_kernel, dim3(blk), dim3(1024), 0, st, a);
-  if (nfold > 0) {
+  if (nrun > 0) {
     SggFoldBwd f[SGG_FOLDB_MAX];
     g = scratch;
-    for (int k = 0; k < nfold; ++k) {
+    for (int k = 0; k < nrun; ++k) {
       f[k] = folds[k];
       f[k].dA_src = g;
       f[k].db_src = g + 2 * folds[k].R;
       g += 3 * (size_t)folds[k].R;
     }
-    fold_bwd_multi(f, nfold, st);
+    fold_bwd_multi(f, nrun, st);
   }
   SGG_RETURN_LAUNCH("sgg_grad_finish");
 }
diff --git a/group-gan-gcn-gat_amd/sgan/_native.py b/group-gan-gcn-gat_amd/sgan/_native.py
--- a/group-gan-gcn-gat_amd/sgan/_native.py
+++ b/group-gan-gcn-gat_amd/sgan/_native.py
@@ -72,6 +72,11 @@
 class Fold(ctypes.Structure):
     _fields_ = [("W", _p), ("ldw", _i), ("R", _i), ("E", _i), ("We", _p), ("be", _p), ("b1", _p), ("b2", _p),
                 ("A", _p), ("bias", _p)]
+
+class AdamFold(ctypes.Structure):
+    _fields_ = [("W", _i), ("We", _i), ("be", _i), ("b1", _i), ("b2", _i), ("ldw", _i), ("R", _i), ("E", _i),
+                ("dA", _p), ("dbias", _p), ("dbias_copy", _p), ("A", _p), ("bias", _p)]
+
 
 RED_MAX = 24
 FOLDB_MAX = 6
@@ -216,9 +221,13 @@
                                   ctypes.POINTER(TrajOut), _sargs, _i, _p]),
     "sgg_grad_finish_losses": (_i, [ctypes.POINTER(Red), _i, ctypes.POINTER(FoldBwd), _i, _p, _sz,
                                     ctypes.POINTER(L2Job), _i, ctypes.POINTER(BceJob), _i, _p]),
+    "sgg_grad_finish_sums": (_i, [ctypes.POINTER(Red), _i, ctypes.POINTER(FoldBwd), _i, _i, _p, _sz,
+                                  ctypes.POINTER(L2Job), _i, ctypes.POINTER(BceJob), _i, _p]),
     "sgg_adam_parts": (_i, [ctypes.c_longlong]),
     "sgg_adam_step": (_i, [_p, _p, _p, _p, _p, _i, ctypes.c_double, ctypes.c_double, ctypes.c_double, _f, _f, _p, _p,
                           _sz, _p]),
+    "sgg_adam_step_folds": (_i, [_p, _p, _p, _p, _p, _i, ctypes.c_double, ctypes.c_double, ctypes.c_double, _f, _f, _p,
+                                _p, _sz, ctypes.POINTER(AdamFold), _i, _p]),
     "sgg_xtw": (_i, [_p, _i, _p, _i, _p, _i, _i, _i, _i, _p, _i, _i, _p, _p, _sz, _p]),
     "sgg_fold_fwd": (_i, [_p, _i, _i, _i, _p, _p, _p, _p, _p, _p, _p]),
     "sgg_fold_fwd_multi": (_i, [ctypes.POINTER(Fold), _i, _p]),
diff --git a/group-gan-gcn-gat_amd/sgan/kernels.py b/group-gan-gcn-gat_amd/sgan/kernels.py
--- a/group-gan-gcn-gat_amd/sgan/kernels.py
+++ b/group-gan-gcn-gat_amd/sgan/kernels.py
@@ -372,7 +372,8 @@
             grad_flush()
 
 
-def grad_flush():
+def grad_flush(take=None):
+    held = []
     if not _PENDING:
         flush_losses()
     while _PENDING:
@@ -389,11 +390,29 @@
         if not _PENDING:
             l2, bce, lkeep = _take_losses()
             keep = keep + lkeep
-        _finish_launch(reds, folds, keep, l2, bce)
-
-
-def _finish_launch(reds_l, folds_l, keep, l2_l=(), bce_l=()):
+        taken = [f for f in folds if take is not None and take(f)]
+        if taken:
+            folds = [f for f in folds if not any(f is g for g in taken)] + taken
+        scratch = _finish_launch(reds, folds, keep, l2, bce, nrun=len(folds) - len(taken))
+        off = 0
+        for f in folds:
+            if any(f is g for g in taken):
+                held.append(HeldFold(f, scratch, off, keep))
+            off += 3 * f.R
+    return held
+
+
+class HeldFold:
+
+    def __init__(self, job, scratch, off, keep):
+        self.job, self.scratch, self.keep = job, scratch, keep
+        self.dA = scratch.data_ptr() + 4 * off
+        self.dbias = self.dA + 8 * job.R
+
+
+def _finish_launch(reds_l, folds_l, keep, l2_l=(), bce_l=(), nrun=None):
     lib = _lib()
+    nrun = len(folds_l) if nrun is None else nrun
     assert len(reds_l) <= N.RED_MAX and len(folds_l) <= N.FOLDB_MAX
     assert len(l2_l) <= N.LOSSJOB_MAX and len(bce_l) <= N.LOSSJOB_MAX
     reds = (N.Red * max(1, len(reds_l)))(*reds_l)
@@ -405,14 +424,15 @@
     scratch = torch.empty(max(1, sum(3 * f.R for f in folds_l)), device=dev, dtype=torch.float32)
 
     def launch(reds=reds, folds=folds, nr=nr, nf=nf, l2=l2, bce=bce, nl=nl, nb=nb, keep=list(keep)):
-        N.check(lib.sgg_grad_finish_losses(reds, nr, folds, nf, N.ptr(scratch), scratch.numel() * 4, l2, nl, bce, nb,
-                                           N.stream_ptr()), "sgg_grad_finish")
+        N.check(lib.sgg_grad_finish_sums(reds, nr, folds, nf, nrun, N.ptr(scratch), scratch.numel() * 4, l2, nl, bce,
+                                         nb, N.stream_ptr()), "sgg_grad_finish")
     launch()
     if timer.active:
         nb = sum(4.0 * r.rows * r.cols for r in reds_l) + sum(4.0 * 3 * f.R * max(f.dA_rows, f.db_rows)
                                                                for f in folds_l)
         timer.add("sgg::grad_finish_kernel", (nr, nf, tuple((r.rows, r.cols) for r in reds_l)), nb / 4.0, nb,
                   launch)
+    return scratch
 
 
 class _XW(torch.autograd.Function):
@@ -643,6 +663,48 @@
     return y
 
 
+ADAM_FOLDS = os.environ.get("SGG_ADAM_FOLDS", "1") != "0"
+ADAM_FOLD_MAX_E, ADAM_FOLD_MAX_R, ADAM_FOLD_LDS = 64, 512, 512 * 17
+
+
+def _job_matches(job, W, We, be, b2):
+    Wo = _owner(W)
+    ptr = lambda t: 0 if t is None else t.data_ptr()
+    return ((job.W or 0) == W.data_ptr() and job.ldw == W.stride(0) and (job.R, job.E) == tuple(W.shape)
+            and (job.We or 0) == We.data_ptr() and (job.be or 0) == be.data_ptr()
+            and (job.dW or 0) == ptr(Wo.grad) and job.lddw == W.stride(0)
+            and (job.dWe or 0) == ptr(We.grad) and (job.dbe or 0) == ptr(be.grad)
+            and (not job.dbias_copy or (b2 is not None and job.dbias_copy == ptr(b2.grad))))
+
+
+def adam_fold_plan(act, specs, jobs=()):
+    idx = {id(p): i for i, p in enumerate(act)}
+    used, plan = set(), []
+    for spec in specs:
+        W, We, be, b1, b2 = spec
+        Wo = _owner(W)
+        ts = [Wo, We, be, b1] + ([b2] if b2 is not None else [])
+        if any(id(t) not in idx for t in ts):
+            continue
+        ii = [idx[id(t)] for t in ts]
+        if len(set(ii)) != len(ii) or used & set(ii) or W.dim() != 2 or Wo.dim() != 2:
+            continue
+        (R, E), ldw = W.shape, Wo.shape[1]
+        if W.data_ptr() != Wo.data_ptr() or tuple(W.stride()) != (ldw, 1) or Wo.shape[0] != R:
+            continue
+        if not (1 <= E <= ADAM_FOLD_MAX_E and 1 <= R <= ADAM_FOLD_MAX_R and R * (E + 1) <= ADAM_FOLD_LDS):
+            continue
+        if tuple(We.shape) != (E, 2) or tuple(be.shape) != (E,) or any(tuple(b.shape) != (R,) for b in ts[3:]):
+            continue
+        if any(t.dtype != torch.float32 or not t.is_contiguous() or t.grad is None
+               or t.grad.dtype != torch.float32 or not t.grad.is_contiguous() for t in ts):
+            continue
+        job = next((j for j in jobs if _job_matches(j, W, We, be, b2)), None)
+        used |= set(ii)
+        plan.append((spec, tuple(ii) + ((-1,) if b2 is None else ()), ldw, job))
+    return plan
+
+
 class ClipAdam:
 
     MAX_TENSORS = 48
@@ -651,6 +713,7 @@
         self.params = [p for p in params]
         self.opt = torch.optim.Adam(self.params, lr=lr, betas=betas, eps=eps, capturable=True)
         self._ws = None
+        self.fold_specs = None
 
     def _state(self, p):
         st = self.opt.state[p]
@@ -678,17 +741,37 @@
     def zero_grad(self, set_to_none=True):
         self.opt.zero_grad(set_to_none=set_to_none)
 
-    def step(self, max_norm=0.0):
+    def _specs(self, act):
+        if not ADAM_FOLDS or self.fold_specs is None or not act or len(act) > self.MAX_TENSORS:
+            return []
+        return self.fold_specs()
+
+    def fold_take(self, max_norm=0.0):
+        if max_norm > 0:
+            return None
+        act = [p for p in self.params if p.grad is not None]
+        specs = self._specs(act)
+        if not specs:
+            return None
+        return lambda job: any(j is not None for _, _, _, j in adam_fold_plan(act, specs, [job]))
+
+    def step(self, max_norm=0.0, folds=(), fuse=True):
         lib = _lib()
         grp = self.opt.param_groups[0]
         act = [p for p in self.params if p.grad is not None]
-        if max_norm > 0:
-            self._launch(lib, act, grp, max_norm)
+        plan = adam_fold_plan(act, self._specs(act) if fuse else [], [h.job for h in folds])
+        for h in folds:
+            if not any(j is h.job for _, _, _, j in plan):
+                j = h.job
+                N.check(lib.sgg_fold_bwd(j.W, j.ldw, j.R, j.E, j.We, j.be, h.dA, h.dbias, j.dW, j.lddw, j.dWe, j.dbe,
+                                         j.dbias_copy, N.stream_ptr()), "sgg_fold_bwd")
+        if max_norm > 0 or plan:
+            self._launch(lib, act, grp, max_norm, plan, folds)
             return
         for i in range(0, len(act), self.MAX_TENSORS):
             self._launch(lib, act[i:i + self.MAX_TENSORS], grp, 0.0)
 
-    def _launch(self, lib, act, grp, max_norm):
+    def _launch(self, lib, act, grp, max_norm, plan=(), held=()):
         import ctypes
         if len(act) > self.MAX_TENSORS:
             raise N.NativeError("ClipAdam: %d tensors with gradients, the fused step takes <= %d (clipping needs "
@@ -708,10 +791,28 @@
         if self._ws is None or self._ws.numel() < parts:
             self._ws = torch.zeros(parts, device=act[0].device, dtype=torch.float32)
         b1, b2 = grp["betas"]
-        N.check(lib.sgg_adam_step(arr(act), arr([p.grad for p in act]), arr([s["exp_avg"] for s in st]),
-                                  arr([s["exp_avg_sq"] for s in st]), numel, n, float(grp["lr"]), float(b1),
-                                  float(b2), float(grp["eps"]), float(max_norm), arr([s["step"] for s in st]),
-                                  N.ptr(self._ws), self._ws.numel() * 4, N.stream_ptr()), "sgg_adam_step")
+        args = (arr(act), arr([p.grad for p in act]), arr([s["exp_avg"] for s in st]),
+                arr([s["exp_avg_sq"] for s in st]), numel, n, float(grp["lr"]), float(b1), float(b2),
+                float(grp["eps"]), float(max_norm), arr([s["step"] for s in st]), N.ptr(self._ws),
+                self._ws.numel() * 4)
+        if not plan:
+            N.check(lib.sgg_adam_step(*args, N.stream_ptr()), "sgg_adam_step")
+            return
+        descs, outs = (N.AdamFold * len(plan))(), []
+        for k, (spec, ii, ldw, job) in enumerate(plan):
+            R, E = spec[0].shape
+            A = torch.empty(R, 2, device=act[0].device, dtype=torch.float32)
+            bias = torch.empty(R, device=act[0].device, dtype=torch.float32)
+            h = next((h for h in held if h.job is job), None) if job is not None and max_norm <= 0 else None
+            descs[k] = N.AdamFold(ii[0], ii[1], ii[2], ii[3], ii[4], ldw, R, E, h.dA if h else None,
+                                  h.dbias if h else None, job.dbias_copy if h else None, N.ptr(A), N.ptr(bias))
+            outs.append((spec, A, bias))
+        N.check(lib.sgg_adam_step_folds(*args, descs, len(plan), N.stream_ptr()), "sgg_adam_step_folds")
+        _fold_purge()
+        for spec, A, bias in outs:
+            key, ver = _fold_key(*spec)
+            refs = tuple(weakref.ref(_owner(t)) if t is not None else None for t in spec)
+            _FOLD_CACHE[key] = (ver, A, bias, (), refs)
 
 
 class OwnershipError(N.NativeError):
diff --git a/group-gan-gcn-gat_amd/sgan/train_step.py b/group-gan-gcn-gat_amd/sgan/train_step.py
--- a/group-gan-gcn-gat_amd/sgan/train_step.py
+++ b/group-gan-gcn-gat_amd/sgan/train_step.py
@@ -160,6 +160,9 @@
         self.d_params = list(D.parameters())
         self.opt_g = self.ops.optimizer(self.g_params, self.args.g_learning_rate)
         self.opt_d = self.ops.optimizer(self.d_params, self.args.d_learning_rate)
+        for opt, mod, enc in ((self.opt_g, G, G), (self.opt_d, D, getattr(D, "encoder", None))):
+            if hasattr(opt, "fold_take") and hasattr(mod, "fold_specs") and getattr(enc, "num_layers", 0) == 1:
+                opt.fold_specs = mod.fold_specs
 
     def _noise(self, S_global, s0, s1):
         G = self.G
@@ -172,14 +175,18 @@
 
     def _finish(self, params, opt, loss_terms, clip):
         K.pooldh_check()
-        K.grad_flush()
+        fused = hasattr(opt, "fold_take") and not self.dp.collective
+        held = K.grad_flush(opt.fold_take(clip) if fused else None)
         grads = [p.grad for p in params if p.grad is not None]
         if self.dp.collective:
             vals = torch.stack([t.detach().reshape(()) for t in loss_terms])
             self.dp.allreduce_(grads + [vals])
         else:
             vals = [t.detach().reshape(()) for t in loss_terms]
-        opt.step(max_norm=clip)
+        if hasattr(opt, "fold_take"):
+            opt.step(max_norm=clip, folds=held, fuse=fused)
+        else:
+            opt.step(max_norm=clip)
         return vals
 
     def _prefix(self, obs_rel, copies):
diff --git a/include/sgg.h b/include/sgg.h
--- a/include/sgg.h
+++ b/include/sgg.h
@@ -241,6 +241,9 @@
 int sgg_grad_finish_losses(const SggRed* reds, int nred, const SggFoldBwd* folds, int nfold, float* scratch,
                            size_t scratch_bytes, const SggL2Job* l2, int nl2, const SggBceJob* bce, int nbce,
                            void* stream);
+int sgg_grad_finish_sums(const SggRed* reds, int nred, const SggFoldBwd* folds, int nfold, int nrun, float* scratch,
+                         size_t scratch_bytes, const SggL2Job* l2, int nl2, const SggBceJob* bce, int nbce,
+                         void* stream);
 
 int sgg_head_ok(int K, int N1);
 int sgg_head_slab_cols(int K, int N1);
@@ -391,6 +394,20 @@
 int sgg_adam_step(float* const* params, float* const* grads, float* const* exp_avg, float* const* exp_avg_sq,
                   const long long* numel, int n, double lr, double beta1, double beta2, float eps, float max_norm,
                   float* const* step, float* ws, size_t ws_bytes, void* stream);
+
+typedef struct {
+  int W, We, be, b1, b2;
+  int ldw, R, E;
+  const float* dA;
+  const float* dbias;
+  float* dbias_copy;
+  float* A;
+  float* bias;
+} SggAdamFold;
+int sgg_adam_step_folds(float* const* params, float* const* grads, float* const* exp_avg, float* const* exp_avg_sq,
+                        const long long* numel, int n, double lr, double beta1, double beta2, float eps,
+                        float max_norm, float* const* step, float* ws, size_t ws_bytes, const SggAdamFold* folds,
+                        int nfolds, void* stream);
 
 #define SGG_GATENC_MAX_HEADS 4
 typedef struct {
```

Result: no change. 144,100 scenes/s (-0.8%).
